# opherlieber/rltime

Measured on AMD Instinct MI355X. Metric: sampled transitions/sec (= learner steps/sec x B x T), IQN-LSTM B=512 T=80 84x84x4, higher is better.
Workload: dtype f32

## Files before the change

include/mirl.h:

```cpp
#ifndef MIRL_H
#define MIRL_H

#include <stdint.h>

#ifdef __cplusplus
extern "C" {
#endif

#define MIRL_OK 0
#define MIRL_NEED_MORE 1
#define MIRL_ERR_ARG (-1)
#define MIRL_ERR_HIP (-2)
#define MIRL_ERR_STATE (-3)
#define MIRL_ERR_NOGPU (-4)

#define MIRL_MODE_UNIFORM 0
#define MIRL_MODE_PER 1

typedef struct mirl_replay mirl_replay;

typedef struct mirl_replay_config {
  int64_t size;
  int32_t num_envs;
  int32_t env_base;
  int32_t frame_bytes;
  int32_t extra_f32;
  int32_t state_f32;
  int32_t has_initials;
  int32_t policy_f32;
  int32_t nstep_train;
  int32_t prefix_steps;
  int32_t nstep_target;
  double  gamma;
  int32_t mode;
  int32_t train_frequency;
  int32_t avoid_episode_crossing;
  int32_t overlap;
  double  alpha, beta, eps, max_weight_factor;
  int32_t beta_anneal_mode;
  double  beta_anneal_to;
  int32_t global_importance_scaling;
  int32_t env_ring_slack;
  int32_t device;
  int32_t acting_priority_init;
  double  acting_vf_eps;
  int32_t stack_planes;
} mirl_replay_config;

typedef struct mirl_ingest {
  int32_t count;
  const int32_t* env_ids_host;
  const uint8_t* frames;
  const float*   extra;
  const float*   state;
  const float*   initials;
  const int32_t* actions;
  const float*   policy;
  const float*   rewards;
  const uint8_t* dones;
  int32_t newest_plane_only;
  int64_t frames_stride;
} mirl_ingest;

typedef struct mirl_batch {
  uint8_t* frames;
  float*   extra;
  float*   state;
  float*   initials;
  float*   returns;
  float*   nsteps;
  float*   masks;
  int64_t* actions;
  float*   policy;
  float*   weights;
  int64_t* loss_indices;
} mirl_batch;

const char* mirl_last_error(void);
int mirl_device_count(void);

int mirl_replay_create(const mirl_replay_config* cfg, mirl_replay** out);
int mirl_replay_destroy(mirl_replay* h);

int mirl_replay_ingest(mirl_replay* h, const mirl_ingest* in, void* stream);
int mirl_replay_ingest_plan(mirl_replay* h, int32_t steps, int32_t count, const int32_t* env_ids_host, void* stream);
int mirl_replay_ingest_planned(mirl_replay* h, int32_t step, const mirl_ingest* in, void* stream);

int mirl_replay_prime_stack(mirl_replay* h, const uint8_t* newest_planes, int64_t stride, void* stream);

int mirl_ingest_fused_set(int32_t on);

int mirl_replay_needed_feed_count(mirl_replay* h, int32_t mbatch, int32_t num_envs, int64_t* out);

int mirl_replay_set_train_quota(mirl_replay* h, int64_t quota);

int mirl_replay_sample(mirl_replay* h, int32_t mbatch, double train_progress,
                       const void* rng_host, uint64_t seed,
                       int32_t* slot, int32_t* env, int64_t* start, int64_t* loss_start,
                       float* weight, double* stats, void* stream);
int mirl_replay_sample_ready(mirl_replay* h, int32_t mbatch, int32_t* ready);
int mirl_replay_sample_skip(mirl_replay* h, int32_t mbatch);
int mirl_replay_tree_root(mirl_replay* h, double* root_dev, void* stream);
int mirl_replay_sample_global(mirl_replay* h, int32_t mbatch_local, int32_t mbatch_global, int32_t rows,
                              int32_t rank, int32_t world, const double* shard_totals,
                              double train_progress, uint64_t seed, int32_t* slot, int32_t* env,
                              int64_t* start, int64_t* loss_start, double* weight_raw,
                              int32_t* stratum, double* stats, void* stream);
int mirl_replay_uniform_total(mirl_replay* h, int64_t* total);

int mirl_replay_state_rows(mirl_replay* h, int32_t* rows, int32_t* overlapped);

int mirl_replay_gather(mirl_replay* h, int32_t mbatch, const int32_t* env,
                       const int64_t* start, const int64_t* loss_start, const float* weight,
                       const mirl_batch* out, void* stream);

int mirl_replay_update_losses(mirl_replay* h, int64_t count, const int64_t* indices,
                              const float* losses, void* stream);

int mirl_replay_save(mirl_replay* h, const char* path_host);
int mirl_replay_load(mirl_replay* h, const char* path_host);

int mirl_replay_profile(mirl_replay* h, int32_t enable, int64_t* launches, double* total_ms);

int mirl_profile_set(int32_t level);
int mirl_profile_collect(int32_t* n_kernels);
int mirl_profile_get(int32_t i, char* name_host, int32_t name_cap, int64_t* calls,
                     double* total_ms, double* algorithmic_bytes);
int mirl_profile_reset(void);
int mirl_profile_get_flop(int32_t i, double* flop);

int mirl_replay_stats(mirl_replay* h, int64_t* total_items, int64_t* active_sequences,
                      int64_t* train_quota, int64_t* tree_capacity, int64_t* n_slots);
int mirl_replay_env_meta(mirl_replay* h, int64_t* first_host, int64_t* count_host);
int mirl_replay_free_slots(mirl_replay* h, int32_t* slots_host, int64_t* n);
int mirl_replay_slot_table(mirl_replay* h, int32_t* slot_env_host, int64_t* slot_base_host);
int mirl_replay_tree_nodes(mirl_replay* h, double* value_host, uint8_t* kind_host, double* min_host);
int mirl_replay_tree_set_leaves(mirl_replay* h, int64_t n, const double* value_host,
                                const uint8_t* kind_host, void* stream);
int mirl_replay_tree_find(mirl_replay* h, int32_t mbatch, const double* uniforms_host,
                          int64_t* idx_host, void* stream);
int mirl_replay_losses_peek(mirl_replay* h, int32_t env_local, int64_t offset, int32_t n, float* out_host);

int mirl_q_target_dqn(int64_t M, int32_t A, const float* q_target, const float* q_select,
                      const float* returns, const float* nsteps, const float* masks,
                      double gamma, double vf_eps, float* targets, void* stream);
int mirl_q_target_iqn(int64_t M, int32_t Nt, int32_t Ns, int32_t A,
                      const float* z_target, const float* z_select,
                      const float* returns, const float* nsteps, const float* masks,
                      double gamma, double vf_eps, float* targets, void* stream);

int mirl_loss_dqn(int64_t M, int32_t A, const float* q, const int64_t* actions,
                  const float* targets, const float* weights, double kappa, int32_t mode,
                  double row_scale, float* row_loss, float* dq, float* td, void* stream);
int mirl_loss_iqn(int64_t M, int32_t N, int32_t Nt, int32_t A, const float* z,
                  const float* taus, const int64_t* actions, const float* targets,
                  const float* weights, double kappa, double row_scale,
                  float* row_loss, float* dz, float* abs_td, void* stream);

int mirl_q_target_c51(int64_t M, int32_t A, int32_t Z, const float* logits_target, const float* logits_select,
                      const float* support, const float* returns, const float* nsteps, const float* masks,
                      double gamma, double vmin, double vmax, double delta_z, int32_t projection,
                      float* targets, void* stream);
int mirl_loss_c51(int64_t M, int32_t A, int32_t Z, const float* logits, const int64_t* actions,
                  const float* targets, const float* weights, int32_t mode, double kappa, double row_scale,
                  float* row_loss, float* dlogits, float* report, void* stream);

int mirl_lstm_cell_fwd(int32_t B, int32_t H, float* gates, const float* c_in, const float* keep_next,
                       float* h_out, float* c_out, float* h_next, float* c_next, void* stream);
int mirl_lstm_seq_supported(int32_t T, int32_t B, int32_t H);
int mirl_lstm_seq_workspace_bytes(int32_t B, int32_t H, int64_t* bytes);
int mirl_lstm_seq_fwd(int32_t T, int32_t B, int32_t H, float* gx, const float* w_hh, const float* h0,
                      const float* c0, const float* keep, float* out, float* c_all, float* hm, float* cm,
                      float* h_last, float* c_last, int32_t save_gates, void* workspace, void* stream);
int mirl_lstm_seq_status(int32_t* status);
int mirl_lstm_seq_fwd_grid(int32_t B, int32_t H, int32_t* workgroups, int64_t* lds_bytes, int32_t* compute_units,
                           int32_t* per_compute_unit);
int mirl_lstm_seq_bwd_supported(int32_t T, int32_t B, int32_t H);
int mirl_lstm_seq_bwd_workspace_bytes(int32_t B, int32_t H, int64_t* bytes);
int mirl_lstm_seq_bwd(int32_t T, int32_t B, int32_t H, float* gates, const float* w_hh, const float* c_all,
                      const float* cm, const float* d_out, const float* keep, void* workspace, void* stream);
int mirl_lstm_cell_bwd(int32_t B, int32_t H, float* gates, const float* c_t, const float* c_in,
                       const float* d_out, const float* dh_rec, float* dc_rec, const float* keep_next,
                       int32_t first, void* stream);

int mirl_frames_to_f32_nhwc(int64_t N, int32_t C, int32_t HW, const uint8_t* src, float scale,
                            float* dst, void* stream);
int mirl_frames_to_f32_nhwc_ex(int64_t N, int32_t C, int32_t HW, const uint8_t* src, float scale,
                               float* dst, int32_t per_wg, int32_t flags, void* stream);

int mirl_conv1_u8_supported(int32_t C, int32_t H, int32_t W, int32_t F, int32_t K, int32_t S);
int mirl_conv1_u8_wpk_floats(int64_t* out);
int mirl_conv1_bf16_set(int32_t mode);
int mirl_conv1_wrw_bf16_set(int32_t mode);
int mirl_conv1_u8_fwd(int64_t N, int32_t H, int32_t W, const uint8_t* x, const float* weight,
                      int64_t ws_o, int64_t ws_c, int64_t ws_h, int64_t ws_w, const float* bias,
                      float scale, float* wpk, float* y, void* stream);
int mirl_conv1_u8_fwd_ex(int64_t N, int32_t H, int32_t W, const uint8_t* x, const float* weight,
                         int64_t ws_o, int64_t ws_c, int64_t ws_h, int64_t ws_w, const float* bias,
                         float scale, float* wpk, float* y, int32_t flags, void* stream);

int mirl_conv1_u8_wrw_scratch_floats(int64_t* out);
int mirl_conv1_u8_wrw(int64_t N, int32_t H, int32_t W, const uint8_t* x, const float* g, float scale,
                      float* scratch, float* dw, int64_t ws_o, int64_t ws_c, int64_t ws_h, int64_t ws_w,
                      void* stream);
int mirl_conv1_u8_wrw_ex(int64_t N, int32_t H, int32_t W, const uint8_t* x, const float* g, float scale,
                         float* scratch, float* dw, int64_t ws_o, int64_t ws_c, int64_t ws_h, int64_t ws_w,
                         int32_t flags, void* stream);
int mirl_conv1_u8_wrw_masked(int64_t N, int32_t H, int32_t W, const uint8_t* x, const float* dy, const float* y, float scale,
                             float* scratch, float* dw, int64_t ws_o, int64_t ws_c, int64_t ws_h, int64_t ws_w,
                             float* db, void* stream);

int mirl_conv2_bwd_data_supported(int32_t C, int32_t F, int32_t K, int32_t S, int32_t IH, int32_t IW,
                                  int32_t OH, int32_t OW);
int mirl_conv2_bwd_data(int64_t N, int32_t OH, int32_t OW, const float* g, const float* weight,
                        int64_t ws_o, int64_t ws_c, int64_t ws_h, int64_t ws_w, float* wpk, float* dx,
                        void* stream);
int mirl_conv2_bwd_data_wpk_floats(int64_t* floats);
int mirl_conv2_bwd_data_ex(int64_t N, int32_t OH, int32_t OW, const float* g, const float* weight, int64_t ws_o,
                           int64_t ws_c, int64_t ws_h, int64_t ws_w, float* wpk, int64_t wpk_floats, float* dx, int32_t pipe,
                           void* stream);
int mirl_conv3_bwd_data_supported(int32_t C, int32_t F, int32_t K, int32_t S, int32_t IH, int32_t IW, int32_t OH, int32_t OW);
int mirl_conv3_bwd_data_wpk_floats(int64_t* floats);
int mirl_conv3_bwd_data(int64_t N, int32_t OH, int32_t OW, const float* g, const float* weight, int64_t ws_o,
                        int64_t ws_c, int64_t ws_h, int64_t ws_w, float* wpk, int64_t wpk_floats, float* dx, void* stream);

int mirl_gemm3_supported(int32_t layout, int64_t M, int64_t N, int64_t K);
int mirl_gemm3_workspace_bytes(int32_t layout, int64_t M, int64_t N, int64_t K, int64_t* bytes);
int mirl_gemm3(int32_t layout, int64_t M, int64_t N, int64_t K, const float* A, int64_t lda,
               const float* B, int64_t ldb, float* C, int64_t ldc, const float* bias, int32_t relu,
               void* workspace, int64_t workspace_bytes, void* stream);
int mirl_gemm3_mid_set(int32_t mode);
int mirl_gemm3_nt_mul(int64_t M, int64_t N, int64_t K, const float* A, int64_t lda, const float* B,
                      int64_t ldb, float* C, int64_t ldc, const float* bias, int32_t relu,
                      const float* mul, int64_t ldmul, int32_t group_shift, float* pre, int64_t ldpre,
                      void* stream);
int mirl_gemm3_head_workspace_bytes(int64_t M, int64_t N, int64_t* bytes);
int mirl_gemm3_nt_head(int64_t M, int64_t N, int64_t K, const float* A, int64_t lda, const float* B, int64_t ldb,
                       float* C, int64_t ldc, const float* bias, int32_t relu, const float* w2, int32_t O,
                       const float* bias2, float* out2, int64_t ldo, void* workspace, int64_t workspace_bytes, void* stream);
int mirl_gemm3_nn_qp_partial_rows(int64_t M, int64_t* rows);
int mirl_gemm3_nn_qp(int64_t M, int64_t N, int64_t K, const float* A, int64_t lda, const float* B, int64_t ldb,
                     const float* emb, int64_t ldemb, const float* x, int64_t ldx, float* d_pre, int64_t ldd,
                     float* dx, int64_t lddx, float* db_partial, void* stream);

int mirl_conv3_fwd_supported(int32_t C, int32_t F, int32_t KH, int32_t KW, int32_t S, int32_t H, int32_t W);
int mirl_conv3_fwd(int64_t N, int32_t H, int32_t W, int32_t C, int32_t F, int32_t KH, int32_t KW, int32_t S,
                   const float* x, const float* w, const float* bias, int32_t relu, float* y, void* stream);

int mirl_conv_wrw_b3_supported(int32_t C, int32_t F, int32_t KH, int32_t KW, int32_t S, int32_t H, int32_t W);
int mirl_conv_wrw_b3_scratch_bytes(int32_t C, int32_t F, int32_t KH, int32_t KW, int64_t* bytes);
int mirl_conv_wrw_b3(int64_t N, int32_t H, int32_t W, int32_t C, int32_t F, int32_t KH, int32_t KW, int32_t S,
                     const float* x, const float* g, void* scratch, int64_t scratch_bytes, float* dw, void* stream);

int mirl_bias_relu_rows(int64_t rows, int32_t C, float* y, const float* bias, void* stream);
int mirl_colsum_blocks(int64_t rows, int32_t C, int32_t* blocks);
int mirl_relu_bwd_bias_rows(int64_t rows, int32_t C, const float* dy, const float* y, float* g,
                            float* db, float* partial, int32_t blocks, void* stream);
int mirl_cos_embed(int64_t rows, int32_t D, const float* tau, const float* freq, float* phi, void* stream);
int mirl_cos_embed_rng(int64_t rows, int32_t D, uint64_t seed, const uint64_t* step, const float* freq,
                       float* phi, float* tau_out, void* stream);
int mirl_iqn_mul_fwd(int64_t M, int32_t N, int32_t C, const float* x, const float* emb, float* out, void* stream);
int mirl_iqn_mul_bwd(int64_t M, int32_t N, int32_t C, const float* g, const float* emb, const float* x,
                     float* d_pre, float* dx, float* db, float* partial, int32_t blocks, void* stream);

int mirl_dueling_tail_bwd(int64_t M, int32_t H1, int32_t Hv, int32_t A, int32_t Q, const float* ga,
                          const float* gv, const float* wo, const float* wq, const float* both,
                          float* g, float* db, float* partial, int32_t blocks, void* stream);
int mirl_dueling_tail_bwd_w(int64_t M, int32_t H1, int32_t Hv, int32_t A, int32_t Q, const float* ga,
                            const float* gv, const float* wo, const float* wq, const float* both, float* g,
                            float* db, float* partial, int32_t blocks, float* dwj, float* partial_w,
                            void* stream);

int mirl_actor_head(int32_t E, int32_t N, int32_t A, const float* adv, const float* val, int32_t Q,
                    const double* eps, const double* expo, double eps_min, const float* u, const int64_t* rnd,
                    int32_t* actions, float* qvalues, float* eps_used, void* stream);
int mirl_actor_head_rng(int32_t E, int32_t N, int32_t A, const float* adv, int32_t adv_pitch, const float* val, int32_t Q,
                        const double* eps, const double* expo, double eps_min, uint64_t rng_seed,
                        const uint64_t* rng_step, int32_t* actions, float* qvalues, float* eps_used, void* stream);
int mirl_actor_head_c51(int32_t E, int32_t A, int32_t Z, const float* adv, int32_t adv_pitch, const float* val,
                        int32_t val_pitch, const float* support, const double* eps, const double* expo, double eps_min,
                        const float* u, const int64_t* rnd, uint64_t rng_seed, const uint64_t* rng_step,
                        int32_t* actions, float* qvalues, float* eps_used, void* stream);
int mirl_stack_shift(int32_t E, int32_t P, int32_t plane_bytes, const uint8_t* in, uint8_t* out,
                     const uint8_t* newest, const uint8_t* dones, void* stream);
#define MIRL_STEP_ADVANCE (~0ull)
int mirl_actor_pre(int32_t E, int32_t H, int32_t A, const float* rewards_raw, const uint8_t* dones,
                   const int32_t* actions, const float* h, const float* c, float* xh_tail, int64_t xh_pitch,
                   float* c_in, float* state_pack, float* initials, float* rewards_out, uint8_t* dones_out,
                   int32_t clip_rewards, float* ep_reward, int32_t* ep_len, float* out_reward, int32_t* out_len,
                   int32_t* action_counts, uint64_t* rng_step, uint64_t step, void* stream);
int mirl_synth_env_step(int32_t E, int64_t frame_bytes, const uint8_t* pool, int32_t pool_n, uint64_t* clock, int32_t slot,
                        uint64_t seed, float p_neg, float p_nonpos, float p_done, uint8_t* obs, float* rewards,
                        uint8_t* dones, void* stream);
int mirl_act_conv_supported(int32_t layer, int32_t Ci, int32_t Co, int32_t k, int32_t stride, int32_t Hi, int32_t Wi);
int mirl_act_conv_fwd(int32_t layer, int64_t frames, int32_t Hi, int32_t Wi, const float* x, const float* w_taps,
                      const float* bias, float* y, int64_t y_frame_pitch, void* stream);
int mirl_act_lstm_supported(int32_t E, int32_t H, int32_t K);
int mirl_act_lstm_workspace_bytes(int32_t E, int32_t H, int32_t K, int64_t* bytes);
int mirl_act_lstm_fwd(int32_t E, int32_t H, int32_t K, const float* xh, int64_t xh_pitch, const float* w, const float* bias,
                      const float* c_in, float* h_out, float* c_out, void* workspace, void* stream);
int mirl_act_embed(int32_t E, int32_t N, int32_t H, int32_t D, const float* h, const float* freq, const float* taus,
                   uint64_t seed, const uint64_t* step, const float* wq, const float* bq, float* x, float* tau_out, void* stream);
int mirl_act_head_supported(int32_t E, int32_t N, int32_t H, int32_t D, int32_t HID, int32_t NO);
int mirl_act_head_parts(int32_t HID, int32_t NO, int32_t* parts, int32_t* pitch);
int mirl_act_head_hidden(int32_t R, int32_t H, int32_t HID, int32_t NO, const float* x, const float* wfc, const float* bfc,
                         const float* wout, float* part, void* stream);
int mirl_act_head_select(int32_t E, int32_t N, int32_t A, int32_t parts, int32_t pitch, const float* part, const float* bout,
                         int32_t has_val, const double* eps, const double* expo, double eps_min, uint64_t rng_seed,
                         const uint64_t* rng_step, int32_t* actions, float* qvalues, void* stream);
int mirl_synth_env_step_pre(int32_t E, int64_t frame_bytes, const uint8_t* pool, int32_t pool_n, uint64_t* clock, int32_t slot,
                            uint64_t seed, float p_neg, float p_nonpos, float p_done, uint8_t* obs, float* rewards,
                            uint8_t* dones, int32_t H, int32_t A, const int32_t* actions, const float* h, const float* c,
                            float* xh_tail, int64_t xh_pitch, float* c_in, float* state_pack, float* initials,
                            float* rewards_out, uint8_t* dones_out, int32_t clip_rewards, float* ep_reward, int32_t* ep_len,
                            float* out_reward, int32_t* out_len, int32_t* action_counts, uint64_t* rng_step, uint64_t step,
                            void* stream);
int mirl_episode_track(int32_t E, int32_t A, const float* rewards, const uint8_t* dones,
                       const int32_t* actions, float* ep_reward, int32_t* ep_len,
                       float* out_reward, int32_t* out_len, int32_t* action_counts, void* stream);

int mirl_copy_bytes(void* dst, const void* src, int64_t bytes, void* stream);
int mirl_copy_bytes_ex(void* dst, const void* src, int64_t bytes, int32_t nt, void* stream);

typedef struct mirl_book mirl_book;
int mirl_book_create(const mirl_replay_config* cfg, mirl_book** out);
int mirl_book_destroy(mirl_book* b);
int mirl_book_ingest(mirl_book* b, int32_t count, const int32_t* env_ids_host);
int mirl_book_stats(mirl_book* b, int64_t* total_items, int64_t* active_sequences,
                    int64_t* train_quota, int64_t* tree_capacity, int64_t* n_slots);
int mirl_book_env_meta(mirl_book* b, int64_t* first_host, int64_t* count_host);
int mirl_book_free_slots(mirl_book* b, int32_t* slots_host, int64_t* n);
int mirl_book_slot_table(mirl_book* b, int32_t* slot_env_host, int64_t* slot_base_host);
int mirl_book_needed_feed_count(mirl_book* b, int32_t mbatch, int32_t num_envs, int64_t* out);
int mirl_book_charge_quota(mirl_book* b, int32_t mbatch);
int mirl_book_uniform_total(mirl_book* b, int64_t* total);
int mirl_book_uniform_map(mirl_book* b, int32_t mbatch, const int64_t* picks_host,
                          int32_t* env_host, int64_t* start_host);
int mirl_emul_build_tree(int64_t capacity, const double* leaf_value, const uint8_t* leaf_kind,
                         double* node_value, uint8_t* node_kind);
int mirl_emul_find(int64_t capacity, const double* node_value, const uint8_t* node_kind,
                   int32_t mbatch, const double* uniforms, int64_t* idx);
int mirl_emul_seq_priority(int32_t nstep_train, double alpha, double max_weight_factor,
                           const float* loss_slots, double* value, uint8_t* kind);

int mirl_adam_clip_workspace_bytes(int32_t count, const int64_t* numel, int64_t* bytes);
int mirl_adam_clip_step(int32_t count, float* const* param, float* const* grad, float* const* exp_avg,
                        float* const* exp_avg_sq, float* const* step, const int64_t* numel, double lr,
                        const float* lr_dev, double beta1, double beta2, double eps, double clip, void* workspace,
                        int64_t workspace_bytes, float* norm_out, void* stream);

#define MIRL_VETO_LOSS 1
#define MIRL_VETO_NORM 2
#define MIRL_VETO_STATUS 4
int mirl_step_guard_open(int32_t* guard, const float* rows, int64_t count, const int32_t* const* status,
                         int32_t n_status, void* stream);
int mirl_adam_clip_step_guarded(int32_t count, float* const* param, float* const* grad, float* const* exp_avg,
                                float* const* exp_avg_sq, float* const* step, const int64_t* numel, double lr,
                                const float* lr_dev, double beta1, double beta2, double eps, double clip, void* workspace,
                                int64_t workspace_bytes, float* norm_out, int32_t* guard, void* stream);
int mirl_replay_update_losses_guarded(mirl_replay* h, int64_t count, const int64_t* indices, const float* losses,
                                      const int32_t* guard, void* stream);
int mirl_lstm_seq_status_device(const int32_t** p);

#ifdef __cplusplus
}
#endif
#endif
```

rltime_amd/_lib.py:

```python
import ctypes as C
import os

import torch

_HERE = os.path.dirname(os.path.abspath(__file__))
LIB_PATH = os.path.join(_HERE, "librltime_hip.so")

MIRL_OK = 0
MIRL_NEED_MORE = 1
MODE_UNIFORM = 0
MODE_PER = 1
INT32_MIN = -2 ** 31


MIRL_OK, MIRL_ERR_ARG, MIRL_ERR_HIP, MIRL_ERR_STATE, MIRL_ERR_NOGPU = 0, -1, -2, -3, -4


class MirlError(RuntimeError):
    code = None


class ReplayConfig(C.Structure):
    _fields_ = [
        ("size", C.c_int64),
        ("num_envs", C.c_int32),
        ("env_base", C.c_int32),
        ("frame_bytes", C.c_int32),
        ("extra_f32", C.c_int32),
        ("state_f32", C.c_int32),
        ("has_initials", C.c_int32),
        ("policy_f32", C.c_int32),
        ("nstep_train", C.c_int32),
        ("prefix_steps", C.c_int32),
        ("nstep_target", C.c_int32),
        ("gamma", C.c_double),
        ("mode", C.c_int32),
        ("train_frequency", C.c_int32),
        ("avoid_episode_crossing", C.c_int32),
        ("overlap", C.c_int32),
        ("alpha", C.c_double),
        ("beta", C.c_double),
        ("eps", C.c_double),
        ("max_weight_factor", C.c_double),
        ("beta_anneal_mode", C.c_int32),
        ("beta_anneal_to", C.c_double),
        ("global_importance_scaling", C.c_int32),
        ("env_ring_slack", C.c_int32),
        ("device", C.c_int32),
        ("acting_priority_init", C.c_int32),
        ("acting_vf_eps", C.c_double),
        ("stack_planes", C.c_int32),
    ]


class Ingest(C.Structure):
    _fields_ = [
        ("count", C.c_int32),
        ("env_ids_host", C.c_void_p),
        ("frames", C.c_void_p),
        ("extra", C.c_void_p),
        ("state", C.c_void_p),
        ("initials", C.c_void_p),
        ("actions", C.c_void_p),
        ("policy", C.c_void_p),
        ("rewards", C.c_void_p),
        ("dones", C.c_void_p),
        ("newest_plane_only", C.c_int32),
        ("frames_stride", C.c_int64),
    ]


class Batch(C.Structure):
    _fields_ = [
        ("frames", C.c_void_p),
        ("extra", C.c_void_p),
        ("state", C.c_void_p),
        ("initials", C.c_void_p),
        ("returns", C.c_void_p),
        ("nsteps", C.c_void_p),
        ("masks", C.c_void_p),
        ("actions", C.c_void_p),
        ("policy", C.c_void_p),
        ("weights", C.c_void_p),
        ("loss_indices", C.c_void_p),
    ]


def _load():
    if not os.path.isfile(LIB_PATH):
        raise MirlError(
            "%s not found: build it with `python -c 'import __graft_entry__ as g; "
            "g.build()'` (rltime_amd/csrc/build.sh). rltime_amd has no CPU "
            "fallback." % LIB_PATH)
    lib = C.CDLL(LIB_PATH)
    lib.mirl_last_error.restype = C.c_char_p
    return lib


lib = _load()

_vp, _i32, _i64, _u64, _f64 = C.c_void_p, C.c_int32, C.c_int64, C.c_uint64, C.c_double
_P = C.POINTER

_SIGNATURES = {
    "mirl_device_count": [],
    "mirl_replay_create": [_P(ReplayConfig), _P(_vp)],
    "mirl_replay_destroy": [_vp],
    "mirl_replay_ingest": [_vp, _P(Ingest), _vp],
    "mirl_replay_ingest_plan": [_vp, _i32, _i32, _vp, _vp],
    "mirl_replay_ingest_planned": [_vp, _i32, _P(Ingest), _vp],
    "mirl_ingest_fused_set": [_i32],
    "mirl_replay_prime_stack": [_vp, _vp, _i64, _vp],
    "mirl_replay_needed_feed_count": [_vp, _i32, _i32, _P(_i64)],
    "mirl_replay_sample": [_vp, _i32, _f64, _vp, _u64, _vp, _vp, _vp, _vp, _vp, _vp, _vp],
    "mirl_replay_sample_ready": [_vp, _i32, _P(_i32)],
    "mirl_replay_sample_skip": [_vp, _i32],
    "mirl_replay_tree_root": [_vp, _vp, _vp],
    "mirl_replay_sample_global": [_vp, _i32, _i32, _i32, _i32, _i32, _vp, _f64, _u64, _vp, _vp, _vp, _vp, _vp, _vp, _vp, _vp],
    "mirl_replay_profile": [_vp, _i32, _P(_i64), _P(_f64)],
    "mirl_profile_set": [_i32],
    "mirl_profile_collect": [_P(_i32)],
    "mirl_profile_get": [_i32, C.c_char_p, _i32, _P(_i64), _P(_f64), _P(_f64)],
    "mirl_profile_get_flop": [_i32, _vp],
    "mirl_profile_reset": [],
    "mirl_replay_save": [_vp, C.c_char_p],
    "mirl_replay_load": [_vp, C.c_char_p],
    "mirl_replay_uniform_total": [_vp, _P(_i64)],
    "mirl_replay_set_train_quota": [_vp, _i64],
    "mirl_replay_state_rows": [_vp, _P(_i32), _P(_i32)],
    "mirl_replay_gather": [_vp, _i32, _vp, _vp, _vp, _vp, _P(Batch), _vp],
    "mirl_replay_update_losses": [_vp, _i64, _vp, _vp, _vp],
    "mirl_replay_stats": [_vp, _P(_i64), _P(_i64), _P(_i64), _P(_i64), _P(_i64)],
    "mirl_replay_env_meta": [_vp, _vp, _vp],
    "mirl_replay_free_slots": [_vp, _vp, _P(_i64)],
    "mirl_replay_slot_table": [_vp, _vp, _vp],
    "mirl_replay_tree_nodes": [_vp, _vp, _vp, _vp],
    "mirl_replay_tree_set_leaves": [_vp, _i64, _vp, _vp, _vp],
    "mirl_replay_tree_find": [_vp, _i32, _vp, _vp, _vp],
    "mirl_replay_losses_peek": [_vp, _i32, _i64, _i32, _vp],
    "mirl_q_target_dqn": [_i64, _i32, _vp, _vp, _vp, _vp, _vp, _f64, _f64, _vp, _vp],
    "mirl_q_target_iqn": [_i64, _i32, _i32, _i32, _vp, _vp, _vp, _vp, _vp, _f64, _f64, _vp, _vp],
    "mirl_loss_dqn": [_i64, _i32, _vp, _vp, _vp, _vp, _f64, _i32, _f64, _vp, _vp, _vp, _vp],
    "mirl_loss_iqn": [_i64, _i32, _i32, _i32, _vp, _vp, _vp, _vp, _vp, _f64, _f64, _vp, _vp, _vp, _vp],
    "mirl_q_target_c51": [_i64, _i32, _i32, _vp, _vp, _vp, _vp, _vp, _vp, _f64, _f64, _f64, _f64, _i32, _vp, _vp],
    "mirl_loss_c51": [_i64, _i32, _i32, _vp, _vp, _vp, _vp, _i32, _f64, _f64, _vp, _vp, _vp, _vp],
    "mirl_actor_head_c51": [_i32, _i32, _i32, _vp, _i32, _vp, _i32, _vp, _vp, _vp, _f64, _vp, _vp, _u64, _vp, _vp, _vp, _vp, _vp],
    "mirl_lstm_cell_fwd": [_i32, _i32, _vp, _vp, _vp, _vp, _vp, _vp, _vp, _vp],
    "mirl_lstm_seq_supported": [_i32, _i32, _i32],
    "mirl_lstm_seq_workspace_bytes": [_i32, _i32, _P(_i64)],
    "mirl_lstm_seq_fwd": [_i32, _i32, _i32, _vp, _vp, _vp, _vp, _vp, _vp, _vp, _vp, _vp, _vp, _vp, _i32, _vp, _vp],
    "mirl_lstm_seq_status": [_P(_i32)],
    "mirl_gemm3_mid_set": [_i32],
    "mirl_lstm_seq_fwd_grid": [_i32, _i32, _P(_i32), _P(_i64), _P(_i32), _P(_i32)],
    "mirl_lstm_seq_bwd_supported": [_i32, _i32, _i32],
    "mirl_lstm_seq_bwd_workspace_bytes": [_i32, _i32, _P(_i64)],
    "mirl_lstm_seq_bwd": [_i32, _i32, _i32, _vp, _vp, _vp, _vp, _vp, _vp, _vp, _vp],
    "mirl_lstm_cell_bwd": [_i32, _i32, _vp, _vp, _vp, _vp, _vp, _vp, _vp, _i32, _vp],
    "mirl_frames_to_f32_nhwc": [_i64, _i32, _i32, _vp, C.c_float, _vp, _vp],
    "mirl_frames_to_f32_nhwc_ex": [_i64, _i32, _i32, _vp, C.c_float, _vp, _i32, _i32, _vp],
    "mirl_conv1_u8_supported": [_i32, _i32, _i32, _i32, _i32, _i32],
    "mirl_conv1_bf16_set": [_i32],
    "mirl_conv1_wrw_bf16_set": [_i32],
    "mirl_conv1_u8_wpk_floats": [_P(_i64)],
    "mirl_conv1_u8_fwd": [_i64, _i32, _i32, _vp, _vp, _i64, _i64, _i64, _i64, _vp, C.c_float, _vp, _vp, _vp],
    "mirl_conv1_u8_fwd_ex": [_i64, _i32, _i32, _vp, _vp, _i64, _i64, _i64, _i64, _vp, C.c_float, _vp, _vp, _i32, _vp],
    "mirl_conv1_u8_wrw_scratch_floats": [_P(_i64)],
    "mirl_conv1_u8_wrw_ex": [_i64, _i32, _i32, _vp, _vp, C.c_float, _vp, _vp, _i64, _i64, _i64, _i64, _i32, _vp],
    "mirl_conv1_u8_wrw_masked": [_i64, _i32, _i32, _vp, _vp, _vp, C.c_float, _vp, _vp, _i64, _i64, _i64, _i64, _vp, _vp],
    "mirl_conv1_u8_wrw": [_i64, _i32, _i32, _vp, _vp, C.c_float, _vp, _vp, _i64, _i64, _i64, _i64, _vp],
    "mirl_conv2_bwd_data_supported": [_i32, _i32, _i32, _i32, _i32, _i32, _i32, _i32],
    "mirl_conv2_bwd_data": [_i64, _i32, _i32, _vp, _vp, _i64, _i64, _i64, _i64, _vp, _vp, _vp],
    "mirl_conv2_bwd_data_wpk_floats": [_P(_i64)],
    "mirl_conv3_bwd_data_supported": [_i32, _i32, _i32, _i32, _i32, _i32, _i32, _i32],
    "mirl_conv3_bwd_data_wpk_floats": [_P(_i64)],
    "mirl_conv3_bwd_data": [_i64, _i32, _i32, _vp, _vp, _i64, _i64, _i64, _i64, _vp, _i64, _vp, _vp],
    "mirl_conv2_bwd_data_ex": [_i64, _i32, _i32, _vp, _vp, _i64, _i64, _i64, _i64, _vp, _i64, _vp, _i32, _vp],
    "mirl_conv3_fwd_supported": [_i32, _i32, _i32, _i32, _i32, _i32, _i32],
    "mirl_conv3_fwd": [_i64, _i32, _i32, _i32, _i32, _i32, _i32, _i32, _vp, _vp, _vp, _i32, _vp, _vp],
    "mirl_conv_wrw_b3_supported": [_i32, _i32, _i32, _i32, _i32, _i32, _i32],
    "mirl_conv_wrw_b3_scratch_bytes": [_i32, _i32, _i32, _i32, _P(_i64)],
    "mirl_conv_wrw_b3": [_i64, _i32, _i32, _i32, _i32, _i32, _i32, _i32, _vp, _vp, _vp, _i64, _vp, _vp],
    "mirl_gemm3_supported": [_i32, _i64, _i64, _i64],
    "mirl_gemm3_workspace_bytes": [_i32, _i64, _i64, _i64, _P(_i64)],
    "mirl_gemm3": [_i32, _i64, _i64, _i64, _vp, _i64, _vp, _i64, _vp, _i64, _vp, _i32, _vp, _i64, _vp],
    "mirl_gemm3_nt_mul": [_i64, _i64, _i64, _vp, _i64, _vp, _i64, _vp, _i64, _vp, _i32, _vp, _i64, _i32, _vp, _i64, _vp],
    "mirl_gemm3_nn_qp_partial_rows": [_i64, _P(_i64)],
    "mirl_gemm3_nn_qp": [_i64, _i64, _i64, _vp, _i64, _vp, _i64, _vp, _i64, _vp, _i64, _vp, _i64, _vp, _i64, _vp, _vp],
    "mirl_gemm3_head_workspace_bytes": [_i64, _i64, _P(_i64)],
    "mirl_gemm3_nt_head": [_i64, _i64, _i64, _vp, _i64, _vp, _i64, _vp, _i64, _vp, _i32, _vp, _i32, _vp, _vp, _i64, _vp, _i64, _vp],
    "mirl_act_conv_supported": [_i32, _i32, _i32, _i32, _i32, _i32, _i32],
    "mirl_act_conv_fwd": [_i32, _i64, _i32, _i32, _vp, _vp, _vp, _vp, _i64, _vp],
    "mirl_act_lstm_supported": [_i32, _i32, _i32],
    "mirl_act_lstm_workspace_bytes": [_i32, _i32, _i32, _P(_i64)],
    "mirl_act_lstm_fwd": [_i32, _i32, _i32, _vp, _i64, _vp, _vp, _vp, _vp, _vp, _vp, _vp],
    "mirl_act_embed": [_i32, _i32, _i32, _i32, _vp, _vp, _vp, _u64, _vp, _vp, _vp, _vp, _vp, _vp],
    "mirl_act_head_supported": [_i32, _i32, _i32, _i32, _i32, _i32],
    "mirl_act_head_parts": [_i32, _i32, _P(_i32), _P(_i32)],
    "mirl_act_head_hidden": [_i32, _i32, _i32, _i32, _vp, _vp, _vp, _vp, _vp, _vp],
    "mirl_act_head_select": [_i32, _i32, _i32, _i32, _i32, _vp, _vp, _i32, _vp, _vp, _f64, _u64, _vp, _vp, _vp, _vp],
    "mirl_bias_relu_rows": [_i64, _i32, _vp, _vp, _vp],
    "mirl_colsum_blocks": [_i64, _i32, _P(_i32)],
    "mirl_relu_bwd_bias_rows": [_i64, _i32, _vp, _vp, _vp, _vp, _vp, _i32, _vp],
    "mirl_cos_embed": [_i64, _i32, _vp, _vp, _vp, _vp],
    "mirl_cos_embed_rng": [_i64, _i32, _u64, _vp, _vp, _vp, _vp, _vp],
    "mirl_adam_clip_workspace_bytes": [_i32, _vp, _vp],
    "mirl_adam_clip_step": [_i32, _vp, _vp, _vp, _vp, _vp, _vp, _f64, _vp, _f64, _f64, _f64, _f64, _vp, _i64, _vp, _vp],
    "mirl_adam_clip_step_guarded": [_i32, _vp, _vp, _vp, _vp, _vp, _vp, _f64, _vp, _f64, _f64, _f64, _f64, _vp, _i64, _vp, _vp, _vp],
    "mirl_step_guard_open": [_vp, _vp, _i64, _vp, _i32, _vp],
    "mirl_replay_update_losses_guarded": [_vp, _i64, _vp, _vp, _vp, _vp],
    "mirl_lstm_seq_status_device": [_P(_vp)],
    "mirl_iqn_mul_fwd": [_i64, _i32, _i32, _vp, _vp, _vp, _vp],
    "mirl_iqn_mul_bwd": [_i64, _i32, _i32, _vp, _vp, _vp, _vp, _vp, _vp, _vp, _i32, _vp],
    "mirl_dueling_tail_bwd": [_i64, _i32, _i32, _i32, _i32, _vp, _vp, _vp, _vp, _vp, _vp, _vp, _vp, _i32, _vp],
    "mirl_dueling_tail_bwd_w": [_i64, _i32, _i32, _i32, _i32, _vp, _vp, _vp, _vp, _vp, _vp, _vp, _vp, _i32, _vp, _vp, _vp],
    "mirl_actor_head": [_i32, _i32, _i32, _vp, _vp, _i32, _vp, _vp, _f64, _vp, _vp, _vp, _vp, _vp, _vp],
    "mirl_actor_head_rng": [_i32, _i32, _i32, _vp, _i32, _vp, _i32, _vp, _vp, _f64, _u64, _vp, _vp, _vp, _vp, _vp],
    "mirl_stack_shift": [_i32, _i32, _i32, _vp, _vp, _vp, _vp, _vp],
    "mirl_synth_env_step": [_i32, _i64, _vp, _i32, _vp, _i32, _u64, C.c_float, C.c_float, C.c_float, _vp, _vp, _vp, _vp],
    "mirl_synth_env_step_pre": [_i32, _i64, _vp, _i32, _vp, _i32, _u64, C.c_float, C.c_float, C.c_float, _vp, _vp, _vp,
                                _i32, _i32, _vp, _vp, _vp, _vp, _i64, _vp, _vp, _vp, _vp, _vp, _i32, _vp, _vp, _vp, _vp, _vp, _vp, _u64, _vp],
    "mirl_actor_pre": [_i32, _i32, _i32, _vp, _vp, _vp, _vp, _vp, _vp, _i64, _vp, _vp, _vp, _vp, _vp, _i32, _vp, _vp, _vp, _vp,
                       _vp, _vp, _u64, _vp],
    "mirl_episode_track": [_i32, _i32, _vp, _vp, _vp, _vp, _vp, _vp, _vp, _vp, _vp],
    "mirl_copy_bytes": [_vp, _vp, _i64, _vp],
    "mirl_copy_bytes_ex": [_vp, _vp, _i64, _i32, _vp],
    "mirl_book_create": [_P(ReplayConfig), _P(_vp)],
    "mirl_book_destroy": [_vp],
    "mirl_book_ingest": [_vp, _i32, _vp],
    "mirl_book_stats": [_vp, _P(_i64), _P(_i64), _P(_i64), _P(_i64), _P(_i64)],
    "mirl_book_env_meta": [_vp, _vp, _vp],
    "mirl_book_free_slots": [_vp, _vp, _P(_i64)],
    "mirl_book_slot_table": [_vp, _vp, _vp],
    "mirl_book_needed_feed_count": [_vp, _i32, _i32, _P(_i64)],
    "mirl_book_charge_quota": [_vp, _i32],
    "mirl_book_uniform_total": [_vp, _P(_i64)],
    "mirl_book_uniform_map": [_vp, _i32, _vp, _vp, _vp],
    "mirl_emul_build_tree": [_i64, _vp, _vp, _vp, _vp],
    "mirl_emul_find": [_i64, _vp, _vp, _i32, _vp, _vp],
    "mirl_emul_seq_priority": [_i32, _f64, _f64, _vp, _P(_f64), _P(C.c_uint8)],
}

for _name, _args in _SIGNATURES.items():
    _fn = getattr(lib, _name)
    _fn.argtypes = _args
    _fn.restype = C.c_int


def last_error():
    return (lib.mirl_last_error() or b"").decode()


def check(rc, what=""):
    if rc < 0:
        err = MirlError("%s failed (%d): %s" % (what or "mirl call", rc, last_error()))
        err.code = int(rc)
        raise err
    return rc


def ptr(t):
    return C.c_void_p(t.data_ptr() if t is not None else None)


def stream():
    return C.c_void_p(torch.cuda.current_stream().cuda_stream)


def device_count():
    return lib.mirl_device_count()


def require_gpu():
    if device_count() <= 0:
        raise MirlError(
            "librltime_hip: no HIP device visible. The rltime_amd hot path runs "
            "only on an AMD GPU (MI355X / gfx950); there is no CPU fallback.")


def profile_table():
    n = C.c_int32()
    check(lib.mirl_profile_collect(C.byref(n)), "mirl_profile_collect")
    out = []
    for i in range(n.value):
        name = C.create_string_buffer(96)
        calls, ms, by = C.c_int64(), C.c_double(), C.c_double()
        check(lib.mirl_profile_get(i, name, 96, C.byref(calls), C.byref(ms), C.byref(by)), "mirl_profile_get")
        fl = C.c_double()
        check(lib.mirl_profile_get_flop(i, C.byref(fl)), "mirl_profile_get_flop")
        out.append({"name": name.value.decode(), "calls": calls.value, "total_ms": ms.value,
                    "algorithmic_bytes": by.value, "flop": fl.value})
    return out


def np_ptr(a):
    return a.ctypes.data_as(C.c_void_p)
```

rltime_amd/csrc/conv_mid.hip:

```cpp
#include "common.hpp"
#include "split3.hpp"
#include <stdlib.h>

namespace mirl {

typedef float cm_f4 __attribute__((ext_vector_type(4)));

constexpr int C2_C = 32, C2_F = 64, C2_K = 4, C2_S = 2;
constexpr int C2_STEPS = 64;
constexpr int C2_WPK = 4 * 2 * C2_STEPS * 64;
constexpr int C2_PP = 68;
constexpr int C2_LD = 6;

__global__ void __launch_bounds__(256)
k_conv2_pack_w(const float* __restrict__ w, int64_t so, int64_t sc, int64_t sh, int64_t sw, float* __restrict__ wpk) {
  const int t = blockIdx.x * 256 + threadIdx.x;
  if (t >= C2_WPK) return;
  const int lane = t & 63, s = (t >> 6) & 63, m = (t >> 12) & 1, cls = t >> 13;
  const int i = lane & 15, kq = lane >> 4;
  const int f = kq * 16 + (s & 15), kh = (cls >> 1) + 2 * (s >> 5), kw = (cls & 1) + 2 * ((s >> 4) & 1);
  const int c = (i >> 2) * 8 + m * 4 + (i & 3);
  wpk[t] = w[f * so + c * sc + kh * sh + kw * sw];
}

template <int FPI>
__global__ void __launch_bounds__(256, 2)
k_conv2_bwd_data(int N, int OH, int OW, unsigned v_magic, const float* __restrict__ g,
                 const float* __restrict__ wpk, float* __restrict__ dx) {
  extern __shared__ __align__(16) float c2_lds[];
  const int tid = threadIdx.x, lane = tid & 63, cls = __builtin_amdgcn_readfirstlane(tid >> 6);
  const int j = lane & 15, kq = lane >> 4;
  const int ph = cls >> 1, pw = cls & 1;
  float wr0[C2_STEPS], wr1[C2_STEPS];
#pragma unroll
  for (int s = 0; s < C2_STEPS; ++s) {
    wr0[s] = wpk[((cls * 2 + 0) * C2_STEPS + s) * 64 + lane];
    wr1[s] = wpk[((cls * 2 + 1) * C2_STEPS + s) * 64 + lane];
  }
  const int PW = OW + 2, rows = FPI * (OH + 1) + 1;
  const int U = OH + 1, V = OW + 1, UV = U * V, IH = 2 * OH + 2, IW = 2 * OW + 2;
  const int pos16 = OH * OW * 16;
  for (int o = tid; o < rows * PW * (C2_PP / 4); o += 256) reinterpret_cast<cm_f4*>(c2_lds)[o] = cm_f4{0.f, 0.f, 0.f, 0.f};
  const int units = (N + FPI - 1) / FPI;
  for (int u0 = blockIdx.x; u0 < units; u0 += gridDim.x) {
    const int n0 = u0 * FPI;
    const int frames = N - n0 < FPI ? N - n0 : FPI;
    __syncthreads();
    {
      const int vecs = frames * pos16;
      const cm_f4* s4 = reinterpret_cast<const cm_f4*>(g + (int64_t)n0 * OH * OW * C2_F);
      for (int o0 = tid; o0 < vecs; o0 += 256 * C2_LD) {
        cm_f4 v[C2_LD];
#pragma unroll
        for (int k = 0; k < C2_LD; ++k) { const int o = o0 + k * 256; v[k] = s4[o < vecs ? o : vecs - 1]; }
#pragma unroll
        for (int k = 0; k < C2_LD; ++k) {
          const int o = o0 + k * 256;
          if (o < vecs) {
            const int f = o >= pos16 ? 1 : 0, r = o - f * pos16, pos = r >> 4, sub = r & 15;
            const int oh2 = pos / OW, ow2 = pos - oh2 * OW;
            *reinterpret_cast<cm_f4*>(c2_lds + ((f * (OH + 1) + 1 + oh2) * PW + 1 + ow2) * C2_PP + sub * 4) = v[k];
          }
        }
      }
    }
    __syncthreads();
    const int pend = frames * UV;
    for (int p0 = 0; p0 < pend; p0 += 16) {
      const int p = p0 + j, pc = p < pend ? p : pend - 1;
      const int f = (FPI > 1 && pc >= UV) ? 1 : 0, r = pc - f * UV;
      const int u = V == 1 ? r : (int)__umulhi((unsigned)r, v_magic), v = r - u * V;
      const float* base = c2_lds + ((f * (OH + 1) + 1 + u) * PW + 1 + v) * C2_PP + kq * 16;
      cm_f4 gq[16];
#pragma unroll
      for (int ab = 0; ab < 4; ++ab) {
        const float* pb = base - ((ab >> 1) * PW + (ab & 1)) * C2_PP;
#pragma unroll
        for (int e = 0; e < 4; ++e) gq[ab * 4 + e] = *reinterpret_cast<const cm_f4*>(pb + e * 4);
      }
      cm_f4 a0 = {0.f, 0.f, 0.f, 0.f}, a1 = {0.f, 0.f, 0.f, 0.f};
#pragma unroll
      for (int s = 0; s < C2_STEPS; ++s) {
        const float val = gq[s >> 2][s & 3];
        a0 = __builtin_amdgcn_mfma_f32_16x16x4f32(wr0[s], val, a0, 0, 0, 0);
        a1 = __builtin_amdgcn_mfma_f32_16x16x4f32(wr1[s], val, a1, 0, 0, 0);
      }
      if (p < pend) {
        cm_f4* dst = reinterpret_cast<cm_f4*>(dx + ((((int64_t)(n0 + f) * IH + 2 * u + ph) * IW) + 2 * v + pw) * C2_C + kq * 8);
        dst[0] = a0; dst[1] = a1;
      }
    }
  }
}

static size_t c2_lds_bytes(int fpi, int OH, int OW) { return (size_t)(fpi * (OH + 1) + 1) * (OW + 2) * C2_PP * 4; }

constexpr int C2B_SLOTS = 4 * 2 * 8;
constexpr int C2B_PF = 6;
constexpr int C2B_WPK_BYTES = C2B_SLOTS * 3 * 64 * 16;

__host__ __device__ inline int c2b_chunk_stride(int npos) { return ((npos + 15) / 16) * 256 + 16; }
__host__ __device__ inline int c2b_half_plane(int npos) { return (4 * c2b_chunk_stride(npos) + 255) / 256 * 256; }

__global__ void __launch_bounds__(256)
k_conv2_pack_w3b(const float* __restrict__ w, int64_t so, int64_t sc, int64_t sh, int64_t sw, uint4* __restrict__ wpk3) {
  const int t = blockIdx.x * 256 + threadIdx.x;
  if (t >= C2B_SLOTS * 64) return;
  const int lane = t & 63, slot = t >> 6, st = slot & 7, m = (slot >> 3) & 1, cls = slot >> 4;
  const int c = 16 * m + (lane & 15), tap = st >> 1;
  const int kh = (cls >> 1) + 2 * (tap >> 1), kw = (cls & 1) + 2 * (tap & 1);
  const int f0 = 32 * (st & 1) + 8 * (lane >> 4);
  float x[2][4];
#pragma unroll
  for (int e = 0; e < 8; ++e) x[e >> 2][e & 3] = w[(f0 + e) * so + c * sc + kh * sh + kw * sw];
  uint2 h0, m0, l0, h1, m1, l1;
  g3_split4(x[0], h0, m0, l0);
  g3_split4(x[1], h1, m1, l1);
  wpk3[(slot * 3 + 0) * 64 + lane] = make_uint4(h0.x, h0.y, h1.x, h1.y);
  wpk3[(slot * 3 + 1) * 64 + lane] = make_uint4(m0.x, m0.y, m1.x, m1.y);
  wpk3[(slot * 3 + 2) * 64 + lane] = make_uint4(l0.x, l0.y, l1.x, l1.y);
}

template <int FPI>
__global__ void __launch_bounds__(512) __attribute__((amdgpu_waves_per_eu(2, 2)))
k_conv2_bwd_data_b3(int N, int OH, int OW, unsigned v_magic, const float* __restrict__ g,
                    const uint4* __restrict__ wpk3, float* __restrict__ dx) {
  extern __shared__ __align__(16) char c2b_lds[];
  const int tid = threadIdx.x, lane = tid & 63, wave = __builtin_amdgcn_readfirstlane(tid >> 6);
  const int cls = wave >> 1, m = wave & 1;
  const int j = lane & 15, kq = lane >> 4;
  const int ph = cls >> 1, pw = cls & 1;
  g3_bf16x8 wr[8][3];
#pragma unroll
  for (int s = 0; s < 8; ++s)
#pragma unroll
    for (int p = 0; p < 3; ++p)
      wr[s][p] = __builtin_bit_cast(g3_bf16x8, wpk3[((((cls * 2 + m) * 8 + s) * 3) + p) * 64 + lane]);
  const int PW = OW + 2, rows = FPI * (OH + 1) + 1;
  const int U = OH + 1, V = OW + 1, UV = U * V, IH = 2 * OH + 2, IW = 2 * OW + 2;
  const int pos16 = OH * OW * 16;
  const int S = c2b_chunk_stride(rows * PW), HP = c2b_half_plane(rows * PW), plane = 2 * HP;
  for (int o = tid; o < 3 * plane / 16; o += 512) reinterpret_cast<uint4*>(c2b_lds)[o] = make_uint4(0u, 0u, 0u, 0u);
  const int units = (N + FPI - 1) / FPI;
  constexpr int PF = C2B_PF;
  const bool pf = FPI * pos16 <= 512 * PF;
  cm_f4 nv[PF];
  auto request = [&](int unit) {
    const int nn0 = unit * FPI;
    const int vecs = (N - nn0 < FPI ? N - nn0 : FPI) * pos16;
    const cm_f4* s4 = reinterpret_cast<const cm_f4*>(g + (int64_t)nn0 * OH * OW * C2_F);
#pragma unroll
    for (int k = 0; k < PF; ++k) { const int o = tid + k * 512; nv[k] = s4[o < vecs ? o : vecs - 1]; }
  };
  auto put = [&](const cm_f4& val, int o) {
    const int f = o >= pos16 ? 1 : 0, r = o - f * pos16, pos = r >> 4, sub = r & 15;
    const int oh2 = pos / OW, ow2 = pos - oh2 * OW;
    const float x[4] = {val.x, val.y, val.z, val.w};
    uint2 hh, mm, ll;
    g3_split4(x, hh, mm, ll);
    const int chunk = sub >> 1, kqw = chunk & 3;
    char* d = c2b_lds + (kqw & 1) * HP + (2 * (chunk >> 2) + (kqw >> 1)) * S + ((f * (OH + 1) + 1 + oh2) * PW + 1 + ow2) * 16 + (sub & 1) * 8;
    *reinterpret_cast<uint2*>(d) = hh;
    *reinterpret_cast<uint2*>(d + plane) = mm;
    *reinterpret_cast<uint2*>(d + 2 * plane) = ll;
  };
  if (pf && (int)blockIdx.x < units) request(blockIdx.x);
  for (int u0 = blockIdx.x; u0 < units; u0 += gridDim.x) {
    const int n0 = u0 * FPI;
    const int frames = N - n0 < FPI ? N - n0 : FPI;
    __syncthreads();
    {
      const int vecs = frames * pos16;
      if (pf) {
#pragma unroll
        for (int k = 0; k < PF; ++k) { const int o = tid + k * 512; if (o < vecs) put(nv[k], o); }
      } else {
        const cm_f4* s4 = reinterpret_cast<const cm_f4*>(g + (int64_t)n0 * OH * OW * C2_F);
        constexpr int LD = 4;
        for (int o0 = tid; o0 < vecs; o0 += 512 * LD) {
          cm_f4 v[LD];
#pragma unroll
          for (int k = 0; k < LD; ++k) { const int o = o0 + k * 512; v[k] = s4[o < vecs ? o : vecs - 1]; }
#pragma unroll
          for (int k = 0; k < LD; ++k) { const int o = o0 + k * 512; if (o < vecs) put(v[k], o); }
        }
      }
    }
    if (pf && u0 + (int)gridDim.x < units) request(u0 + gridDim.x);
    g3_barrier();
    const int pend = frames * UV;
    int f, u, v;
    auto locate = [&](int p0) -> const char* {
      const int p = p0 + j, pc = p < pend ? p : pend - 1;
      f = (FPI > 1 && pc >= UV) ? 1 : 0;
      const int r = pc - f * UV;
      u = V == 1 ? r : (int)__umulhi((unsigned)r, v_magic);
      v = r - u * V;
      return c2b_lds + (kq & 1) * HP + (kq >> 1) * S + ((f * (OH + 1) + 1 + u) * PW + 1 + v) * 16;
    };
    auto load_half = [&](g3_bf16x8 (&b)[4][3], const char* base, int hs) {
#pragma unroll
      for (int q = 0; q < 4; ++q) {
        const int s = hs * 4 + q;
        const char* pb = base - (((s >> 2) & 1) * PW + ((s >> 1) & 1)) * 16 + (s & 1) * 2 * S;
        b[q][0] = *reinterpret_cast<const g3_bf16x8*>(pb);
        b[q][1] = *reinterpret_cast<const g3_bf16x8*>(pb + plane);
        b[q][2] = *reinterpret_cast<const g3_bf16x8*>(pb + 2 * plane);
      }
    };
    auto mfma_half = [&](g3_f32x4 acc, const g3_bf16x8 (&b)[4][3], int hs) -> g3_f32x4 {
#pragma unroll
      for (int q = 0; q < 4; ++q) {
        const int s = hs * 4 + q;
        acc = __builtin_amdgcn_mfma_f32_16x16x32_bf16(wr[s][2], b[q][0], acc, 0, 0, 0);
        acc = __builtin_amdgcn_mfma_f32_16x16x32_bf16(wr[s][0], b[q][2], acc, 0, 0, 0);
        acc = __builtin_amdgcn_mfma_f32_16x16x32_bf16(wr[s][1], b[q][1], acc, 0, 0, 0);
        acc = __builtin_amdgcn_mfma_f32_16x16x32_bf16(wr[s][1], b[q][0], acc, 0, 0, 0);
        acc = __builtin_amdgcn_mfma_f32_16x16x32_bf16(wr[s][0], b[q][1], acc, 0, 0, 0);
        acc = __builtin_amdgcn_mfma_f32_16x16x32_bf16(wr[s][0], b[q][0], acc, 0, 0, 0);
      }
      return acc;
    };
    g3_bf16x8 b0[4][3], b1[4][3];
    const char* base = locate(0);
    load_half(b0, base, 0);
    for (int p0 = 0; p0 < pend; p0 += 16) {
      load_half(b1, base, 1);
      float* dst = dx + ((((int64_t)(n0 + f) * IH + 2 * u + ph) * IW) + 2 * v + pw) * C2_C + 16 * m + 4 * kq;
      const bool live = p0 + j < pend;
      __builtin_amdgcn_sched_barrier(0);
      g3_f32x4 acc = {0.f, 0.f, 0.f, 0.f};
      acc = mfma_half(acc, b0, 0);
      __builtin_amdgcn_sched_barrier(0);
      if (p0 + 16 < pend) {
        base = locate(p0 + 16);
        load_half(b0, base, 0);
      }
      __builtin_amdgcn_sched_barrier(0);
      acc = mfma_half(acc, b1, 1);
      __builtin_amdgcn_sched_barrier(0);
      if (live) *reinterpret_cast<g3_f32x4*>(dst) = acc;
    }
  }
}

static size_t c2b_lds_bytes(int fpi, int OH, int OW) { return (size_t)3 * 2 * c2b_half_plane((fpi * (OH + 1) + 1) * (OW + 2)); }

constexpr int C3B_C = 64, C3B_F = 64, C3B_K = 3;
constexpr int C3B_HS = 9;
constexpr int C3B_SLOTS = 4 * 2 * C3B_HS;
constexpr int C3B_WPK_BYTES = C3B_SLOTS * 3 * 64 * 16;
constexpr int C3B_MAXT = 11;

__global__ void __launch_bounds__(256)
k_conv3_pack_w3b(const float* __restrict__ w, int64_t so, int64_t sc, int64_t sh, int64_t sw, uint4* __restrict__ wpk3) {
  const int t = blockIdx.x * 256 + threadIdx.x;
  if (t >= C3B_SLOTS * 64) return;
  const int lane = t & 63, slot = t >> 6, q = slot % C3B_HS, kh2 = (slot / C3B_HS) & 1, ct = slot / (2 * C3B_HS);
  const int st = kh2 * C3B_HS + q, tap = st >> 1, kh = tap / C3B_K, kw = tap - kh * C3B_K;
  const int c = 16 * ct + (lane & 15), f0 = 32 * (st & 1) + 8 * (lane >> 4);
  float x[2][4];
#pragma unroll
  for (int e = 0; e < 8; ++e) x[e >> 2][e & 3] = w[(f0 + e) * so + c * sc + kh * sh + kw * sw];
  uint2 h0, m0, l0, h1, m1, l1;
  g3_split4(x[0], h0, m0, l0);
  g3_split4(x[1], h1, m1, l1);
  wpk3[(slot * 3 + 0) * 64 + lane] = make_uint4(h0.x, h0.y, h1.x, h1.y);
  wpk3[(slot * 3 + 1) * 64 + lane] = make_uint4(m0.x, m0.y, m1.x, m1.y);
  wpk3[(slot * 3 + 2) * 64 + lane] = make_uint4(l0.x, l0.y, l1.x, l1.y);
}

template <int FPI>
__global__ void __launch_bounds__(512) __attribute__((amdgpu_waves_per_eu(2, 2)))
k_conv3_bwd_data_b3(int N, int OH, int OW, unsigned iw_magic, const float* __restrict__ g, const uint4* __restrict__ wpk3,
                    float* __restrict__ dx) {
  extern __shared__ __align__(16) char c3b_lds[];
  const int tid = threadIdx.x, lane = tid & 63, wave = __builtin_amdgcn_readfirstlane(tid >> 6);
  const int ct = wave >> 1, kh2 = wave & 1;
  const int j = lane & 15, kq = lane >> 4;
  g3_bf16x8 wr[C3B_HS][3];
#pragma unroll
  for (int q = 0; q < C3B_HS; ++q)
#pragma unroll
    for (int p = 0; p < 3; ++p)
      wr[q][p] = __builtin_bit_cast(g3_bf16x8, wpk3[((((ct * 2 + kh2) * C3B_HS + q) * 3) + p) * 64 + lane]);
  const int IH = OH + 2, IW = OW + 2, IHW = IH * IW, PW = OW + 4, rows = FPI * (OH + 2) + 2;
  const int pos16 = OH * OW * 16;
  const int S = c2b_chunk_stride(rows * PW), HP = c2b_half_plane(rows * PW), plane = 2 * HP;
  int tsh[C3B_HS], fsh[C3B_HS];
#pragma unroll
  for (int q = 0; q < C3B_HS; ++q) {
    const int st = kh2 * C3B_HS + q, tap = st >> 1, kh = tap / C3B_K, kw = tap - kh * C3B_K;
    tsh[q] = (kh * PW + kw) * 16;
    fsh[q] = (st & 1) * 2 * S;
  }
  for (int o = tid; o < 3 * plane / 16; o += 512) reinterpret_cast<uint4*>(c3b_lds)[o] = make_uint4(0u, 0u, 0u, 0u);
  const int units = (N + FPI - 1) / FPI;
  bool first = true;
  for (int u0 = blockIdx.x; u0 < units; u0 += gridDim.x) {
    const int n0 = u0 * FPI;
    const int frames = N - n0 < FPI ? N - n0 : FPI;
    __syncthreads();
    if (!first) {
      for (int o = tid; o < 4 * C3B_MAXT * 64; o += 512) reinterpret_cast<uint4*>(c3b_lds)[o] = make_uint4(0u, 0u, 0u, 0u);
      __syncthreads();
    }
    first = false;
    {
      const int vecs = frames * pos16;
      const cm_f4* s4 = reinterpret_cast<const cm_f4*>(g + (int64_t)n0 * OH * OW * C3B_F);
      constexpr int LD = 4;
      for (int o0 = tid; o0 < vecs; o0 += 512 * LD) {
        cm_f4 v[LD];
#pragma unroll
        for (int k = 0; k < LD; ++k) { const int o = o0 + k * 512; v[k] = s4[o < vecs ? o : vecs - 1]; }
#pragma unroll
        for (int k = 0; k < LD; ++k) {
          const int o = o0 + k * 512;
          if (o < vecs) {
            const int f = o / pos16, r = o - f * pos16, pos = r >> 4, sub = r & 15;
            const int oh2 = pos / OW, ow2 = pos - oh2 * OW;
            const float x[4] = {v[k].x, v[k].y, v[k].z, v[k].w};
            uint2 hh, mm, ll;
            g3_split4(x, hh, mm, ll);
            const int chunk = sub >> 1, kqw = chunk & 3;
            char* d = c3b_lds + (kqw & 1) * HP + (2 * (chunk >> 2) + (kqw >> 1)) * S + ((f * (OH + 2) + 2 + oh2) * PW + 2 + ow2) * 16 + (sub & 1) * 8;
            *reinterpret_cast<uint2*>(d) = hh;
            *reinterpret_cast<uint2*>(d + plane) = mm;
            *reinterpret_cast<uint2*>(d + 2 * plane) = ll;
          }
        }
      }
    }
    __syncthreads();
    const int pend = frames * IHW;
    g3_f32x4 acc[C3B_MAXT];
#pragma unroll
    for (int t = 0; t < C3B_MAXT; ++t) {
      acc[t] = g3_f32x4{0.f, 0.f, 0.f, 0.f};
      if (t * 16 < pend) {
        const int p = t * 16 + j, pc = p < pend ? p : pend - 1;
        const int f = pc / IHW, r = pc - f * IHW;
        const int y = (int)__umulhi((unsigned)r, iw_magic), x = r - y * IW;
        const char* base = c3b_lds + (kq & 1) * HP + (kq >> 1) * S + ((f * (OH + 2) + 2 + y) * PW + 2 + x) * 16;
        g3_bf16x8 b[C3B_HS][3];
#pragma unroll
        for (int q = 0; q < C3B_HS; ++q) {
          const char* pb = base - tsh[q] + fsh[q];
          b[q][0] = *reinterpret_cast<const g3_bf16x8*>(pb);
          b[q][1] = *reinterpret_cast<const g3_bf16x8*>(pb + plane);
          b[q][2] = *reinterpret_cast<const g3_bf16x8*>(pb + 2 * plane);
        }
        g3_f32x4 a = {0.f, 0.f, 0.f, 0.f};
#pragma unroll
        for (int q = 0; q < C3B_HS; ++q) {
          a = __builtin_amdgcn_mfma_f32_16x16x32_bf16(wr[q][2], b[q][0], a, 0, 0, 0);
          a = __builtin_amdgcn_mfma_f32_16x16x32_bf16(wr[q][0], b[q][2], a, 0, 0, 0);
          a = __builtin_amdgcn_mfma_f32_16x16x32_bf16(wr[q][1], b[q][1], a, 0, 0, 0);
          a = __builtin_amdgcn_mfma_f32_16x16x32_bf16(wr[q][1], b[q][0], a, 0, 0, 0);
          a = __builtin_amdgcn_mfma_f32_16x16x32_bf16(wr[q][0], b[q][1], a, 0, 0, 0);
          a = __builtin_amdgcn_mfma_f32_16x16x32_bf16(wr[q][0], b[q][0], a, 0, 0, 0);
        }
        acc[t] = a;
      }
    }
    __syncthreads();
    g3_f32x4* xb = reinterpret_cast<g3_f32x4*>(c3b_lds) + (ct * C3B_MAXT) * 64 + lane;
    if (kh2 == 1) {
#pragma unroll
      for (int t = 0; t < C3B_MAXT; ++t) if (t * 16 < pend) xb[t * 64] = acc[t];
    }
    __syncthreads();
    if (kh2 == 0) {
#pragma unroll
      for (int t = 0; t < C3B_MAXT; ++t) {
        const int p = t * 16 + j;
        if (p < pend) {
          const int f = p / IHW, r = p - f * IHW;
          *reinterpret_cast<g3_f32x4*>(dx + ((int64_t)(n0 + f) * IHW + r) * C3B_C + 16 * ct + 4 * kq) = acc[t] + xb[t * 64];
        }
      }
    }
  }
}

static size_t c3b_lds_bytes(int fpi, int OH, int OW) {
  const size_t planes = (size_t)3 * 2 * c2b_half_plane((fpi * (OH + 2) + 2) * (OW + 4)), xchg = (size_t)4 * C3B_MAXT * 1024;
  return planes > xchg ? planes : xchg;
}

struct BwdDataLaunch {
  const char *pack_name, *name;
  double pack_bytes, bytes, flop;
  unsigned pack_grid;
  int fpi;
  size_t lds, lds_limit;
  int grid_cap, block, magic_div;
};
template <typename WPK>
static int bwd_data_launch(const BwdDataLaunch& c, void (*pack)(const float*, int64_t, int64_t, int64_t, int64_t, WPK*),
                           void (*k2)(int, int, int, unsigned, const float*, const WPK*, float*),
                           void (*k1)(int, int, int, unsigned, const float*, const WPK*, float*), int64_t N, int32_t OH, int32_t OW,
                           const float* g, const float* weight, int64_t ws_o, int64_t ws_c, int64_t ws_h, int64_t ws_w, float* wpk,
                           float* dx, hipStream_t st) {
  {
    ProfScope ps(c.pack_name, c.pack_bytes, st);
    hipLaunchKernelGGL(pack, dim3(c.pack_grid), dim3(256), 0, st, weight, ws_o, ws_c, ws_h, ws_w, reinterpret_cast<WPK*>(wpk));
    MIRL_LAUNCH_CHECK();
  }
  const auto k = c.fpi == 2 ? k2 : k1;
  if (c.lds_limit) { if (int rc = raise_lds_limit(k, c.lds_limit)) return rc; }
  ProfScope ps(c.name, c.bytes, st, c.flop);
  hipLaunchKernelGGL(k, dim3(capped_grid((N + c.fpi - 1) / c.fpi, c.grid_cap)), dim3(c.block), c.lds, st, (int)N, OH, OW,
                     magic_u32(c.magic_div), g, reinterpret_cast<const WPK*>(wpk), dx);
  MIRL_LAUNCH_CHECK();
  return MIRL_OK;
}

}

extern "C" int mirl_conv2_bwd_data_supported(int32_t C, int32_t F, int32_t K, int32_t S, int32_t IH, int32_t IW, int32_t OH, int32_t OW) {
  using namespace mirl;
  if (C != C2_C || F != C2_F || K != C2_K || S != C2_S || OH < 1 || OW < 1) return 0;
  if (IH != 2 * OH + 2 || IW != 2 * OW + 2) return 0;
  return c2_lds_bytes(1, OH, OW) <= 64 * 1024 ? 1 : 0;
}

extern "C" int mirl_conv2_bwd_data(int64_t N, int32_t OH, int32_t OW, const float* g, const float* weight, int64_t ws_o,
                                   int64_t ws_c, int64_t ws_h, int64_t ws_w, float* wpk, float* dx, void* stream) {
  using namespace mirl;
  if (N <= 0 || N >= (1LL << 30) || !g || !weight || !wpk || !dx) return fail(MIRL_ERR_ARG, "bad conv2_bwd_data arguments");
  if (!mirl_conv2_bwd_data_supported(C2_C, C2_F, C2_K, C2_S, 2 * OH + 2, 2 * OW + 2, OH, OW))
    return fail(MIRL_ERR_ARG, "conv2_bwd_data: unsupported shape");
  if (!aligned16(g, dx, wpk)) return fail(MIRL_ERR_ARG, "conv2_bwd_data: pointers must be 16-byte aligned");
  BwdDataLaunch c;
  c.pack_name = "k_conv2_pack_w"; c.pack_bytes = 2.0 * C2_WPK * 4; c.pack_grid = (C2_WPK + 255) / 256;
  c.fpi = (N >= 1024 && c2_lds_bytes(2, OH, OW) <= 64 * 1024) ? 2 : 1;
  c.lds = c2_lds_bytes(c.fpi, OH, OW); c.lds_limit = 0;
  c.grid_cap = 512; c.block = 256; c.magic_div = OW + 1;
  c.name = "k_conv2_bwd_data"; c.bytes = (double)N * ((double)OH * OW * C2_F * 4 + (double)(2 * OH + 2) * (2 * OW + 2) * C2_C * 4);
  c.flop = (double)N * OH * OW * 2.0 * C2_K * C2_K * C2_C * C2_F;
  return bwd_data_launch<float>(c, k_conv2_pack_w, k_conv2_bwd_data<2>, k_conv2_bwd_data<1>, N, OH, OW, g, weight, ws_o, ws_c, ws_h, ws_w, wpk,
                                dx, (hipStream_t)stream);
}

extern "C" int mirl_conv2_bwd_data_wpk_floats(int64_t* floats) {
  if (!floats) return mirl::fail(MIRL_ERR_ARG, "conv2_bwd_data_wpk_floats: null out");
  *floats = mirl::C2B_WPK_BYTES / 4 > mirl::C2_WPK ? mirl::C2B_WPK_BYTES / 4 : mirl::C2_WPK;
  return MIRL_OK;
}

extern "C" int mirl_conv2_bwd_data_ex(int64_t N, int32_t OH, int32_t OW, const float* g, const float* weight, int64_t ws_o,
                                      int64_t ws_c, int64_t ws_h, int64_t ws_w, float* wpk, int64_t wpk_floats, float* dx, int32_t pipe, void* stream) {
  using namespace mirl;
  if (wpk_floats < (pipe == 1 ? C2B_WPK_BYTES / 4 : C2_WPK)) return fail(MIRL_ERR_ARG, "conv2_bwd_data_ex: wpk smaller than mirl_conv2_bwd_data_wpk_floats()");
  if (pipe == 0) return mirl_conv2_bwd_data(N, OH, OW, g, weight, ws_o, ws_c, ws_h, ws_w, wpk, dx, stream);
  if (pipe != 1) return fail(MIRL_ERR_ARG, "conv2_bwd_data_ex: pipe is 0 (f32) or 1 (split bf16)");
  if (N <= 0 || N >= (1LL << 30) || !g || !weight || !wpk || !dx) return fail(MIRL_ERR_ARG, "bad conv2_bwd_data arguments");
  if (!mirl_conv2_bwd_data_supported(C2_C, C2_F, C2_K, C2_S, 2 * OH + 2, 2 * OW + 2, OH, OW) || c2b_lds_bytes(1, OH, OW) > 160 * 1024)
    return fail(MIRL_ERR_ARG, "conv2_bwd_data: unsupported shape");
  if (!aligned16(g, dx, wpk)) return fail(MIRL_ERR_ARG, "conv2_bwd_data: pointers must be 16-byte aligned");
  BwdDataLaunch c;
  c.pack_name = "k_conv2_pack_w3b"; c.pack_bytes = 4.0 * C2_WPK + C2B_WPK_BYTES; c.pack_grid = (C2B_SLOTS * 64 + 255) / 256;
  c.fpi = (N >= 512 && c2b_lds_bytes(2, OH, OW) <= 160 * 1024) ? 2 : 1;
  c.lds = c2b_lds_bytes(c.fpi, OH, OW); c.lds_limit = 160 * 1024;
  c.grid_cap = 256; c.block = 512; c.magic_div = OW + 1;
  c.name = "k_conv2_bwd_data_b3"; c.bytes = (double)N * ((double)OH * OW * C2_F * 4 + (double)(2 * OH + 2) * (2 * OW + 2) * C2_C * 4);
  c.flop = (double)N * OH * OW * 2.0 * C2_K * C2_K * C2_C * C2_F;
  return bwd_data_launch<uint4>(c, k_conv2_pack_w3b, k_conv2_bwd_data_b3<2>, k_conv2_bwd_data_b3<1>, N, OH, OW, g, weight, ws_o, ws_c, ws_h, ws_w,
                                wpk, dx, (hipStream_t)stream);
}


extern "C" int mirl_conv3_bwd_data_supported(int32_t C, int32_t F, int32_t K, int32_t S, int32_t IH, int32_t IW, int32_t OH, int32_t OW) {
  using namespace mirl;
  if (C != C3B_C || F != C3B_F || K != C3B_K || S != 1 || OH < 1 || OW < 1) return 0;
  if (IH != OH + 2 || IW != OW + 2) return 0;
  if (IH * IW > 16 * C3B_MAXT) return 0;
  return c3b_lds_bytes(1, OH, OW) <= 150 * 1024 ? 1 : 0;
}

extern "C" int mirl_conv3_bwd_data_wpk_floats(int64_t* floats) {
  if (!floats) return mirl::fail(MIRL_ERR_ARG, "conv3_bwd_data_wpk_floats: null out");
  *floats = mirl::C3B_WPK_BYTES / 4;
  return MIRL_OK;
}

extern "C" int mirl_conv3_bwd_data(int64_t N, int32_t OH, int32_t OW, const float* g, const float* weight, int64_t ws_o,
                                   int64_t ws_c, int64_t ws_h, int64_t ws_w, float* wpk, int64_t wpk_floats, float* dx, void* stream) {
  using namespace mirl;
  if (N <= 0 || N >= (1LL << 30) || !g || !weight || !wpk || !dx) return fail(MIRL_ERR_ARG, "bad conv3_bwd_data arguments");
  if (wpk_floats < C3B_WPK_BYTES / 4) return fail(MIRL_ERR_ARG, "conv3_bwd_data: wpk smaller than mirl_conv3_bwd_data_wpk_floats()");
  if (!mirl_conv3_bwd_data_supported(C3B_C, C3B_F, C3B_K, 1, OH + 2, OW + 2, OH, OW)) return fail(MIRL_ERR_ARG, "conv3_bwd_data: unsupported shape");
  if (!aligned16(g, dx, wpk)) return fail(MIRL_ERR_ARG, "conv3_bwd_data: pointers must be 16-byte aligned");
  const int IHW = (OH + 2) * (OW + 2);
  BwdDataLaunch c;
  c.pack_name = "k_conv3_pack_w3b"; c.pack_bytes = 4.0 * C3B_F * C3B_C * 9 + C3B_WPK_BYTES; c.pack_grid = (C3B_SLOTS * 64 + 255) / 256;
  c.fpi = (N >= 512 && 2 * IHW <= 16 * C3B_MAXT && c3b_lds_bytes(2, OH, OW) <= 150 * 1024) ? 2 : 1;
  c.lds = c3b_lds_bytes(c.fpi, OH, OW); c.lds_limit = 150 * 1024;
  c.grid_cap = 256; c.block = 512; c.magic_div = OW + 2;
  c.name = "k_conv3_bwd_data_b3"; c.bytes = (double)N * 4.0 * C3B_F * ((double)OH * OW + (double)IHW);
  c.flop = (double)N * OH * OW * 2.0 * C3B_K * C3B_K * C3B_C * C3B_F;
  return bwd_data_launch<uint4>(c, k_conv3_pack_w3b, k_conv3_bwd_data_b3<2>, k_conv3_bwd_data_b3<1>, N, OH, OW, g, weight, ws_o, ws_c, ws_h, ws_w,
                                wpk, dx, (hipStream_t)stream);
}
```

rltime_amd/csrc/gemm3.hip:

```cpp
#include "common.hpp"
#include "split3.hpp"
#include <stdlib.h>

namespace mirl {

struct G3Args {
  const float* A; const float* B; float* C; const float* bias;
  int64_t M, N, K;
  int64_t lda, ldb, ldc;
  int relu;
  int mt, nt;
  int splits;
  int steps_per_split;
  const float* mul; int64_t ldmul; int mul_shift;
  float* pre; int64_t ldpre;
  int vec_ok;
  const float* w2; float* part;
  float* gsum; int64_t ldgsum;
};


template <bool KC>
struct G3Loader {
  const float* p[2];
  int64_t step;
  int64_t ld;
  int lds_off;
  __device__ __forceinline__ void init(const float* base, int64_t ld_, int64_t row0, int64_t rows, int64_t k0, int t) {
    ld = ld_;
    if (KC) {
      const int r = t >> 2, kq = t & 3;
#pragma unroll
      for (int h = 0; h < 2; ++h) {
        int64_t row = row0 + r + 128 * h; if (row > rows - 1) row = rows - 1;
        p[h] = base + row * ld + k0 + kq * 4;
      }
      step = 16;
      lds_off = r * G3_PITCH + kq * 8;
    } else {
      const int kq = t >> 7, r = t & 127;
#pragma unroll
      for (int h = 0; h < 2; ++h) {
        int64_t row = row0 + r + 128 * h; if (row > rows - 1) row = rows - 1;
        p[h] = base + (k0 + kq * 4) * ld + row;
      }
      step = 16 * ld;
      lds_off = r * G3_PITCH + kq * 8;
    }
  }
  __device__ __forceinline__ void load(float (&v)[2][4]) {
#pragma unroll
    for (int h = 0; h < 2; ++h) {
      if (KC) {
        const float4 q = *reinterpret_cast<const float4*>(p[h]);
        v[h][0] = q.x; v[h][1] = q.y; v[h][2] = q.z; v[h][3] = q.w;
      } else {
#pragma unroll
        for (int e = 0; e < 4; ++e) v[h][e] = p[h][e * ld];
      }
      p[h] += step;
    }
  }
  __device__ __forceinline__ void store(char* planes, const float (&v)[2][4]) const {
#pragma unroll
    for (int h = 0; h < 2; ++h) {
      uint2 a, b, c;
      g3_split4(v[h], a, b, c);
      char* d = planes + lds_off + h * 128 * G3_PITCH;
      *reinterpret_cast<uint2*>(d) = a;
      *reinterpret_cast<uint2*>(d + G3_PLANE) = b;
      *reinterpret_cast<uint2*>(d + 2 * G3_PLANE) = c;
    }
  }
};

template <int TI>
__device__ __forceinline__ void g3_compute(const char* stage, g3_f32x16 (&acc)[TI][2], int a_off, int b_off) {
  const char* pa = stage + a_off;
  const char* pb = stage + 3 * G3_PLANE + b_off;
  constexpr int PA[6] = {2, 0, 1, 1, 0, 0};
  constexpr int PB[6] = {0, 2, 1, 0, 1, 0};
  g3_bf16x8 b[3][2];
#pragma unroll
  for (int p = 0; p < 3; ++p)
#pragma unroll
    for (int j = 0; j < 2; ++j) b[p][j] = *reinterpret_cast<const g3_bf16x8*>(pb + p * G3_PLANE + j * 32 * G3_PITCH);
  constexpr int IW = TI >= 2 ? 2 : 1;
#pragma unroll
  for (int ih = 0; ih < TI / IW; ++ih) {
    g3_bf16x8 a[3][IW];
#pragma unroll
    for (int p = 0; p < 3; ++p)
#pragma unroll
      for (int i = 0; i < IW; ++i) a[p][i] = *reinterpret_cast<const g3_bf16x8*>(pa + p * G3_PLANE + (ih * IW + i) * 32 * G3_PITCH);
#pragma unroll
    for (int c = 0; c < 6; ++c)
#pragma unroll
      for (int i = 0; i < IW; ++i)
#pragma unroll
        for (int j = 0; j < 2; ++j) acc[ih * IW + i][j] = g3_mfma(a[PA[c]][i], b[PB[c]][j], acc[ih * IW + i][j]);
  }
}


template <bool AKC, bool BKC, int EP, bool VEC, bool NARROW = false>
__global__ void __launch_bounds__(512)
k_gemm3(G3Args g) {
  constexpr int TI = NARROW ? 1 : 4;
  extern __shared__ __attribute__((aligned(16))) char g3_lds[];
  const int t = threadIdx.x, lane = t & 63, wave = t >> 6;
  const int b = blockIdx.x, xcd = b & 7, l = b >> 3, L = gridDim.x >> 3;
  const int64_t nk_all = g.K / 16;
  const int E = g.splits > 1 ? l + 1 : ((g.mt + 7) / 8) * g.nt;
  int split = 0;
  int64_t ks0 = 0, nk = nk_all;

  const int wu = __builtin_amdgcn_readfirstlane(wave);
  const int wm = NARROW ? 0 : (wu & 1), wn = NARROW ? 0 : (wu >> 1);
  const int row_w = NARROW ? wu * 32 : wm * 128;
  const int a_off = (row_w + (lane & 31)) * G3_PITCH + (lane >> 5) * 16;
  const int b_off = (wn * 64 + (lane & 31)) * G3_PITCH + (lane >> 5) * 16;
  const bool stage_first = (wu >> 2) & 1;

  int e = l, it = 0, jt = 0;
  if (g.splits > 1) {
    const int tiles = g.mt * g.nt, tile = l % tiles;
    split = xcd + 8 * (l / tiles);
    it = tile / g.nt; jt = tile % g.nt;
    ks0 = (int64_t)split * g.steps_per_split;
    nk = nk_all - ks0; if (nk > g.steps_per_split) nk = g.steps_per_split;
    if (nk < 0) nk = 0;
  } else {
    for (; e < E; e += L) { jt = e % g.nt; it = (e / g.nt) * 8 + xcd; if (it < g.mt) break; }
    if (e >= E) return;
  }

  G3Loader<AKC> la; G3Loader<BKC> lb;
  float va[2][4], vb[2][4];
  la.init(g.A, g.lda, (int64_t)it * 256, g.M, ks0 * 16, t);
  lb.init(g.B, g.ldb, (int64_t)jt * 256, g.N, ks0 * 16, t);
  if (nk > 0) { la.load(va); lb.load(vb); }

  g3_f32x16 acc[TI][2];
  while (true) {
    const int64_t m0 = (int64_t)it * 256, n0 = (int64_t)jt * 256;
#pragma unroll
    for (int i = 0; i < TI; ++i)
#pragma unroll
      for (int j = 0; j < 2; ++j)
#pragma unroll
        for (int r = 0; r < 16; ++r) acc[i][j][r] = 0.0f;

    if (nk > 0) {
      la.store(g3_lds, va); lb.store(g3_lds + 3 * G3_PLANE, vb);
      if (nk > 1) { la.load(va); lb.load(vb); }
    }
    g3_barrier();
    for (int64_t k = 0; k < nk; ++k) {
      const char* cur = g3_lds + (k & 1) * G3_STAGE;
      char* nxt = g3_lds + ((k + 1) & 1) * G3_STAGE;
      if (stage_first) {
        if (k + 1 < nk) { la.store(nxt, va); lb.store(nxt + 3 * G3_PLANE, vb); }
        if (k + 2 < nk) { la.load(va); lb.load(vb); }
      }
      __builtin_amdgcn_s_setprio(1);
      g3_compute<TI>(cur, acc, a_off, b_off);
      __builtin_amdgcn_s_setprio(0);
      if (!stage_first) {
        if (k + 1 < nk) { la.store(nxt, va); lb.store(nxt + 3 * G3_PLANE, vb); }
        if (k + 2 < nk) { la.load(va); lb.load(vb); }
      }
      g3_barrier();
    }

    bool more = false;
    if (g.splits <= 1) {
      for (e += L; e < E; e += L) { jt = e % g.nt; it = (e / g.nt) * 8 + xcd; if (it < g.mt) break; }
      more = e < E;
      if (more) {
        la.init(g.A, g.lda, (int64_t)it * 256, g.M, 0, t);
        lb.init(g.B, g.ldb, (int64_t)jt * 256, g.N, 0, t);
        la.load(va); lb.load(vb);
      }
    }

    float* C = g.C + (g.splits > 1 ? (int64_t)split * g.M * g.N : 0);
    if (VEC) {
      float* tl = reinterpret_cast<float*>(g3_lds) + wu * (64 * G3_EPITCH);
      constexpr int HALVES = NARROW ? 1 : 2, II = NARROW ? 1 : 2, QN = NARROW ? 8 : 16;
      float* w2l = reinterpret_cast<float*>(g3_lds) + 8 * (64 * G3_EPITCH);
      float bj[2] = {0.f, 0.f};
      g3_f32x4 sb = {0.f, 0.f, 0.f, 0.f};
      if (EP == 2) {
        const int64_t wc = n0 + (t & 63) * 4;
        float4 w = make_float4(0.f, 0.f, 0.f, 0.f);
        if (wc < g.N) w = *reinterpret_cast<const float4*>(g.w2 + (int64_t)(t >> 6) * g.N + wc);
        *reinterpret_cast<float4*>(w2l + (t >> 6) * 256 + (t & 63) * 4) = w;
#pragma unroll
        for (int j = 0; j < 2; ++j) {
          const int64_t cj = n0 + wn * 64 + j * 32 + (lane & 31);
          bj[j] = (g.bias && cj < g.N) ? g.bias[cj] : 0.f;
        }
#pragma unroll
        for (int i = 0; i < TI; ++i)
#pragma unroll
          for (int j = 0; j < 2; ++j)
#pragma unroll
            for (int r = 0; r < 16; ++r) {
              float v = acc[i][j][r] + bj[j];
              acc[i][j][r] = (g.relu && !(v > 0.f)) ? 0.f : v;
            }
        g3_barrier();
      }
#pragma unroll
      for (int h = 0; h < HALVES; ++h) {
#pragma unroll
        for (int ii = 0; ii < II; ++ii)
#pragma unroll
          for (int j = 0; j < 2; ++j)
#pragma unroll
            for (int r = 0; r < 16; ++r)
              tl[(ii * 32 + (r & 3) + 8 * (r >> 2) + 4 * (lane >> 5)) * G3_EPITCH + j * 32 + (lane & 31)] = acc[II * h + ii][j][r];
        asm volatile("s_waitcnt lgkmcnt(0)" ::: "memory");
        const int c4 = lane & 15;
        const int64_t col = n0 + wn * 64 + c4 * 4;
        float4 bv = make_float4(0.f, 0.f, 0.f, 0.f);
        if (EP != 2 && g.bias && col < g.N) {
          bv = *reinterpret_cast<const float4*>(g.bias + col);
        }
        if (EP == 2) {
          const int rg = lane & 15, cq = lane >> 4;
          const int64_t cb = (n0 >> 6) + wn;
#pragma unroll 1
          for (int ip = 0; ip < 2; ++ip) {
            float ps[2][8];
#pragma unroll
            for (int i = 0; i < 2; ++i)
#pragma unroll
              for (int o = 0; o < 8; ++o) ps[i][o] = 0.f;
#pragma unroll 1
            for (int c = 0; c < 4; ++c) {
              asm volatile("" ::: "memory");
              float4 dv[2];
#pragma unroll
              for (int i = 0; i < 2; ++i) dv[i] = *reinterpret_cast<const float4*>(tl + (rg + 16 * (2 * ip + i)) * G3_EPITCH + cq * 16 + c * 4);
#pragma unroll
              for (int o = 0; o < 8; ++o) {
                const float4 w = *reinterpret_cast<const float4*>(w2l + o * 256 + wn * 64 + cq * 16 + c * 4);
#pragma unroll
                for (int i = 0; i < 2; ++i)
                  ps[i][o] = fmaf(dv[i].w, w.w, fmaf(dv[i].z, w.z, fmaf(dv[i].y, w.y, fmaf(dv[i].x, w.x, ps[i][o]))));
              }
            }
#pragma unroll
            for (int i = 0; i < 2; ++i)
#pragma unroll
              for (int o = 0; o < 8; ++o) {
                float v = ps[i][o];
                v += __shfl_xor(v, 16);
                v += __shfl_xor(v, 32);
                ps[i][o] = v;
              }
            if (cq == 0) {
#pragma unroll
              for (int i = 0; i < 2; ++i) {
                const int64_t row = m0 + row_w + h * 64 + rg + 16 * (2 * ip + i);
                if (row < g.M) {
                  float* d = g.part + (cb * g.M + row) * 8;
                  *reinterpret_cast<float4*>(d) = make_float4(ps[i][0], ps[i][1], ps[i][2], ps[i][3]);
                  *reinterpret_cast<float4*>(d + 4) = make_float4(ps[i][4], ps[i][5], ps[i][6], ps[i][7]);
                }
              }
            }
          }
        }
        float4 mg0 = make_float4(0.f, 0.f, 0.f, 0.f), mg1 = mg0;
        const bool hoisted = (EP == 1 && g.mul_shift >= 5) || EP == 3;
        if ((EP == 1 || EP == 3) && hoisted) {
          const int64_t rb = m0 + row_w + h * 64 + (lane >> 4);
          const int64_t r0 = rb < g.M ? rb : g.M - 1, r1 = rb + 32 < g.M ? rb + 32 : g.M - 1;
          const int64_t cc = col < g.N ? col : 0;
          mg0 = *reinterpret_cast<const float4*>(g.mul + (r0 >> g.mul_shift) * g.ldmul + cc);
          mg1 = *reinterpret_cast<const float4*>(g.mul + (r1 >> g.mul_shift) * g.ldmul + cc);
        }
        if (EP == 3) {
          const float4 mgs[2] = {mg0, mg1};
#pragma unroll
          for (int gq = 0; gq < 2; ++gq) {
            g3_f32x4 ev[8];
#pragma unroll
            for (int u = 0; u < 8; ++u) {
              const int64_t row = m0 + row_w + h * 64 + (gq * 8 + u) * 4 + (lane >> 4);
              const int64_t rr = row < g.M ? row : g.M - 1, cc = col < g.N ? col : 0;
              ev[u] = __builtin_nontemporal_load(reinterpret_cast<const g3_f32x4*>(g.pre + rr * g.ldpre + cc));
            }
            g3_f32x4 sg = {0.f, 0.f, 0.f, 0.f};
            const g3_f32x4 xm = {mgs[gq].x, mgs[gq].y, mgs[gq].z, mgs[gq].w};
#pragma unroll
            for (int u = 0; u < 8; ++u) {
              const int rl = (gq * 8 + u) * 4 + (lane >> 4);
              const int64_t row = m0 + row_w + h * 64 + rl;
              const float4 t4 = *reinterpret_cast<const float4*>(tl + rl * G3_EPITCH + c4 * 4);
              const g3_f32x4 v = {t4.x, t4.y, t4.z, t4.w};
              if (row < g.M && col < g.N) {
                g3_f32x4 d = v * xm;
                d.x = ev[u].x > 0.f ? d.x : 0.f; d.y = ev[u].y > 0.f ? d.y : 0.f;
                d.z = ev[u].z > 0.f ? d.z : 0.f; d.w = ev[u].w > 0.f ? d.w : 0.f;
                __builtin_nontemporal_store(d, reinterpret_cast<g3_f32x4*>(C + row * g.ldc + col));
                sg += v * ev[u];
                sb += d;
              }
            }
#pragma unroll
            for (int e = 0; e < 4; ++e) {
              float v = sg[e];
              v += __shfl_xor(v, 16);
              v += __shfl_xor(v, 32);
              sg[e] = v;
            }
            const int64_t row0 = m0 + row_w + h * 64 + gq * 32;
            if ((lane >> 4) == 0 && row0 < g.M && col < g.N)
              *reinterpret_cast<g3_f32x4*>(g.gsum + (row0 >> 5) * g.ldgsum + col) = sg;
          }
        }
#pragma unroll
        for (int q = 0; q < QN; ++q) {
          const int rl = q * 4 + (lane >> 4);
          const int64_t row = m0 + row_w + h * 64 + rl;
          if (EP == 3) break;
          if (EP == 2 && !g.C) break;
          float4 v = *reinterpret_cast<const float4*>(tl + rl * G3_EPITCH + c4 * 4);
          if (row < g.M && col < g.N) {
            if (EP != 2) {
              v.x += bv.x; v.y += bv.y; v.z += bv.z; v.w += bv.w;
              if (g.relu) { v.x = v.x > 0.f ? v.x : 0.f; v.y = v.y > 0.f ? v.y : 0.f; v.z = v.z > 0.f ? v.z : 0.f; v.w = v.w > 0.f ? v.w : 0.f; }
            }
            if (EP == 1) {
              if (g.pre) __builtin_nontemporal_store(g3_f32x4{v.x, v.y, v.z, v.w}, reinterpret_cast<g3_f32x4*>(g.pre + row * g.ldpre + col));
              float4 m;
              if (hoisted) m = q < 8 ? mg0 : mg1;
              else m = *reinterpret_cast<const float4*>(g.mul + (row >> g.mul_shift) * g.ldmul + col);
              v.x *= m.x; v.y *= m.y; v.z *= m.z; v.w *= m.w;
            }
            __builtin_nontemporal_store(g3_f32x4{v.x, v.y, v.z, v.w}, reinterpret_cast<g3_f32x4*>(C + row * g.ldc + col));
          }
        }
        asm volatile("s_waitcnt lgkmcnt(0)" ::: "memory");
      }
      if (EP == 3) {
#pragma unroll
        for (int e = 0; e < 4; ++e) {
          float v = sb[e];
          v += __shfl_xor(v, 16);
          v += __shfl_xor(v, 32);
          sb[e] = v;
        }
        const int64_t col = n0 + wn * 64 + (lane & 15) * 4;
        if ((lane >> 4) == 0 && col < g.N)
          *reinterpret_cast<g3_f32x4*>(g.part + ((m0 >> 8) * 2 + wm) * g.N + col) = sb;
      }
      if (more) g3_barrier();
    } else {
#pragma unroll
      for (int j = 0; j < 2; ++j) {
        const int64_t col = n0 + wn * 64 + j * 32 + (lane & 31);
        const bool col_ok = col < g.N;
        const float bv = (g.bias && col_ok) ? g.bias[col] : 0.0f;
#pragma unroll
        for (int i = 0; i < TI; ++i) {
          const int64_t rb = m0 + row_w + i * 32 + 4 * (lane >> 5);
#pragma unroll
          for (int r = 0; r < 16; ++r) {
            const int64_t row = rb + (r & 3) + 8 * (r >> 2);
            if (!(col_ok && row < g.M)) continue;
            float v = acc[i][j][r] + bv;
            if (g.relu) v = v > 0.0f ? v : 0.0f;
            if (EP == 1) {
              if (g.pre) __builtin_nontemporal_store(v, g.pre + row * g.ldpre + col);
              v *= g.mul[(row >> g.mul_shift) * g.ldmul + col];
            }
            __builtin_nontemporal_store(v, C + row * g.ldc + col);
          }
        }
      }
    }
    if (!more) break;
  }
}


constexpr int G3M_BROWS = 128;
constexpr int G3M_BPLANE = G3M_BROWS * G3_PITCH;
constexpr int G3M_STAGE = 3 * G3_PLANE + 3 * G3M_BPLANE;
constexpr int G3M_LDS = 2 * G3M_STAGE;
constexpr int G3M_EPITCH = 36;

__global__ void __launch_bounds__(512)
k_gemm3_mid(G3Args g) {
  extern __shared__ __attribute__((aligned(16))) char g3_lds[];
  const int t = threadIdx.x, lane = t & 63;
  const int wu = __builtin_amdgcn_readfirstlane(t >> 6);
  const int wm = wu & 1, wn = wu >> 1;
  const int b = blockIdx.x, xcd = b & 7, l = b >> 3;
  const int jt = l % g.nt, it = (l / g.nt) * 8 + xcd;
  if (it >= g.mt) return;
  const int64_t m0 = (int64_t)it * 256, n0 = (int64_t)jt * G3M_BROWS;
  const int64_t nk = g.K / 16;

  G3Loader<true> la;
  la.init(g.A, g.lda, m0, g.M, 0, t);
  const int rb = t >> 2, kq = t & 3;
  int64_t brow = n0 + rb; if (brow > g.N - 1) brow = g.N - 1;
  const float* pb = g.B + brow * g.ldb + kq * 4;
  const int b_lds = rb * G3_PITCH + kq * 8;
  float va[2][4], vb[4];
  auto load_b = [&]() { const float4 q = *reinterpret_cast<const float4*>(pb); vb[0] = q.x; vb[1] = q.y; vb[2] = q.z; vb[3] = q.w; pb += 16; };
  auto store_b = [&](char* planes) {
    uint2 h, m, lo;
    g3_split4(vb, h, m, lo);
    *reinterpret_cast<uint2*>(planes + b_lds) = h;
    *reinterpret_cast<uint2*>(planes + G3M_BPLANE + b_lds) = m;
    *reinterpret_cast<uint2*>(planes + 2 * G3M_BPLANE + b_lds) = lo;
  };
  const int a_off = (wm * 128 + (lane & 31)) * G3_PITCH + (lane >> 5) * 16;
  const int b_off = (wn * 32 + (lane & 31)) * G3_PITCH + (lane >> 5) * 16;
  const bool stage_first = (wu >> 2) & 1;

  g3_f32x16 acc[4];
#pragma unroll
  for (int i = 0; i < 4; ++i)
#pragma unroll
    for (int r = 0; r < 16; ++r) acc[i][r] = 0.0f;
  constexpr int PA[6] = {2, 0, 1, 1, 0, 0};
  constexpr int PB[6] = {0, 2, 1, 0, 1, 0};

  if (nk > 0) { la.load(va); load_b(); la.store(g3_lds, va); store_b(g3_lds + 3 * G3_PLANE); }
  if (nk > 1) { la.load(va); load_b(); }
  g3_barrier();
  for (int64_t k = 0; k < nk; ++k) {
    const char* cur = g3_lds + (k & 1) * G3M_STAGE;
    char* nxt = g3_lds + ((k + 1) & 1) * G3M_STAGE;
    if (stage_first) {
      if (k + 1 < nk) { la.store(nxt, va); store_b(nxt + 3 * G3_PLANE); }
      if (k + 2 < nk) { la.load(va); load_b(); }
    }
    {
      const char* pa = cur + a_off;
      const char* pbf = cur + 3 * G3_PLANE + b_off;
      g3_bf16x8 bf[3];
#pragma unroll
      for (int p = 0; p < 3; ++p) bf[p] = *reinterpret_cast<const g3_bf16x8*>(pbf + p * G3M_BPLANE);
      __builtin_amdgcn_s_setprio(1);
#pragma unroll
      for (int ih = 0; ih < 2; ++ih) {
        g3_bf16x8 a[3][2];
#pragma unroll
        for (int p = 0; p < 3; ++p)
#pragma unroll
          for (int i = 0; i < 2; ++i) a[p][i] = *reinterpret_cast<const g3_bf16x8*>(pa + p * G3_PLANE + (ih * 2 + i) * 32 * G3_PITCH);
#pragma unroll
        for (int c = 0; c < 6; ++c)
#pragma unroll
          for (int i = 0; i < 2; ++i) acc[ih * 2 + i] = g3_mfma(a[PA[c]][i], bf[PB[c]], acc[ih * 2 + i]);
      }
      __builtin_amdgcn_s_setprio(0);
    }
    if (!stage_first) {
      if (k + 1 < nk) { la.store(nxt, va); store_b(nxt + 3 * G3_PLANE); }
      if (k + 2 < nk) { la.load(va); load_b(); }
    }
    g3_barrier();
  }

  float* tl = reinterpret_cast<float*>(g3_lds) + wu * (32 * G3M_EPITCH);
  const int c4 = lane & 7;
  const int64_t col = n0 + wn * 32 + c4 * 4;
  float4 bv = make_float4(0.f, 0.f, 0.f, 0.f);
  if (g.bias && col < g.N) bv = *reinterpret_cast<const float4*>(g.bias + col);
#pragma unroll
  for (int i = 0; i < 4; ++i) {
#pragma unroll
    for (int r = 0; r < 16; ++r)
      tl[((r & 3) + 8 * (r >> 2) + 4 * (lane >> 5)) * G3M_EPITCH + (lane & 31)] = acc[i][r];
    asm volatile("s_waitcnt lgkmcnt(0)" ::: "memory");
#pragma unroll
    for (int q = 0; q < 4; ++q) {
      const int rl = q * 8 + (lane >> 3);
      const int64_t row = m0 + wm * 128 + i * 32 + rl;
      float4 v = *reinterpret_cast<const float4*>(tl + rl * G3M_EPITCH + c4 * 4);
      if (row < g.M && col < g.N) {
        v.x += bv.x; v.y += bv.y; v.z += bv.z; v.w += bv.w;
        if (g.relu) { v.x = v.x > 0.f ? v.x : 0.f; v.y = v.y > 0.f ? v.y : 0.f; v.z = v.z > 0.f ? v.z : 0.f; v.w = v.w > 0.f ? v.w : 0.f; }
        *reinterpret_cast<float4*>(g.C + row * g.ldc + col) = v;
      }
    }
    asm volatile("s_waitcnt lgkmcnt(0)" ::: "memory");
  }
}

__global__ void __launch_bounds__(256)
k_gemm3_reduce(const float* __restrict__ partial, int splits, int64_t M, int64_t N, float* __restrict__ out, int64_t ldc) {
  const int64_t n4 = N >> 2;
  const int64_t total = M * n4;
  for (int64_t i = (int64_t)blockIdx.x * blockDim.x + threadIdx.x; i < total; i += (int64_t)gridDim.x * blockDim.x) {
    const int64_t row = i / n4, c4 = i - row * n4;
    float4 s = make_float4(0.f, 0.f, 0.f, 0.f);
    for (int k = 0; k < splits; ++k) {
      const float4 v = *reinterpret_cast<const float4*>(partial + ((int64_t)k * M + row) * N + c4 * 4);
      s.x += v.x; s.y += v.y; s.z += v.z; s.w += v.w;
    }
    *reinterpret_cast<float4*>(out + row * ldc + c4 * 4) = s;
  }
}

__global__ void __launch_bounds__(256)
k_g3_head_reduce(const float* __restrict__ part, int ncb, int64_t M, int O, const float* __restrict__ bias2,
                 float* __restrict__ out, int64_t ldo) {
  for (int64_t i = (int64_t)blockIdx.x * 256 + threadIdx.x; i < M * 2; i += (int64_t)gridDim.x * 256) {
    const int64_t row = i >> 1;
    const int half = (int)(i & 1);
    float4 sum = make_float4(0.f, 0.f, 0.f, 0.f);
    for (int cb = 0; cb < ncb; ++cb) {
      const float4 v = *reinterpret_cast<const float4*>(part + ((int64_t)cb * M + row) * 8 + half * 4);
      sum.x += v.x; sum.y += v.y; sum.z += v.z; sum.w += v.w;
    }
    const float r[4] = {sum.x, sum.y, sum.z, sum.w};
#pragma unroll
    for (int e = 0; e < 4; ++e) {
      const int o = half * 4 + e;
      if (o < O) out[row * ldo + o] = r[e] + (bias2 ? bias2[o] : 0.f);
    }
  }
}

static int g_g3_mid_mode = -1;

static int g3_splits(int64_t M, int64_t N, int64_t K) {
  const int64_t tiles = ((M + 255) / 256) * ((N + 255) / 256);
  int64_t s = 8 * ((256 + 8 * tiles - 1) / (8 * tiles));
  const int64_t nk = K / 16;
  while (s > 8 && nk / s < 64) s -= 8;
  return (int)s;
}

}

extern "C" int mirl_gemm3_supported(int32_t layout, int64_t M, int64_t N, int64_t K) {
  if (layout < 0 || layout > 2) return 0;
  if (M < 1 || N < 1 || K < 16 || (K % 16)) return 0;
  if (M >= (1LL << 31) || N >= (1LL << 31)) return 0;
  if (layout == 2) {
    if (N % 4) return 0;
    if (K / 16 < 8) return 0;
  }
  return 1;
}

extern "C" int mirl_gemm3_workspace_bytes(int32_t layout, int64_t M, int64_t N, int64_t K, int64_t* bytes) {
  using namespace mirl;
  if (!bytes) return fail(MIRL_ERR_ARG, "gemm3_workspace_bytes: null out");
  if (!mirl_gemm3_supported(layout, M, N, K)) return fail(MIRL_ERR_ARG, "gemm3: unsupported layout / shape");
  *bytes = layout == 2 ? (int64_t)g3_splits(M, N, K) * M * N * (int64_t)sizeof(float) : 0;
  return MIRL_OK;
}

namespace mirl {
struct G3Opt {
  const float* mul = nullptr; int64_t ldmul = 0; int32_t mul_shift = 0;
  float* pre = nullptr; int64_t ldpre = 0;
  const float* w2 = nullptr; float* part = nullptr;
  float* gsum = nullptr; int64_t ldgsum = 0;
};

struct G3Kernel { const void* fn; const char* name; };
static G3Kernel g3_kernel(int layout, int vec, bool mul, bool w2, bool gsum, bool narrow) {
  static const void* const plain[4][2] = {{(const void*)k_gemm3<true, true, 0, false>, (const void*)k_gemm3<true, true, 0, true>},
                                          {(const void*)k_gemm3<true, false, 0, false>, (const void*)k_gemm3<true, false, 0, true>},
                                          {nullptr , (const void*)k_gemm3<false, false, 0, true>},
                                          {(const void*)k_gemm3<true, true, 1, false>, (const void*)k_gemm3<true, true, 1, true>}};
  static const char* const names[4] = {"k_gemm3_nt", "k_gemm3_nn", "k_gemm3_tn", "k_gemm3_nt_mul"};
  if (gsum) return {(const void*)k_gemm3<true, false, 3, true>, "k_gemm3_nn_qp"};
  if (w2) return {(const void*)k_gemm3<true, true, 2, true>, "k_gemm3_nt_head"};
  if (narrow) return {(const void*)k_gemm3<false, false, 0, true, true>, "k_gemm3_tn"};
  const int which = mul ? 3 : layout;
  return {plain[which][vec], names[which]};
}
}

static int g3_launch(int32_t layout, int64_t M, int64_t N, int64_t K, const float* A, int64_t lda, const float* B,
                     int64_t ldb, float* C, int64_t ldc, const float* bias, int32_t relu, void* workspace,
                     int64_t workspace_bytes, void* stream, const mirl::G3Opt& o = mirl::G3Opt()) {
  using namespace mirl;
  if (!mirl_gemm3_supported(layout, M, N, K)) return fail(MIRL_ERR_ARG, "gemm3: unsupported layout / shape");
  if (!A || !B || (!C && !o.w2)) return fail(MIRL_ERR_ARG, "gemm3: null operand");
  const bool akc = layout != 2, bkc = layout == 0;
  if (akc && ((lda % 4) || !aligned16(A) || lda < K)) return fail(MIRL_ERR_ARG, "gemm3: A must be 16-byte aligned with lda % 4 == 0");
  if (bkc && ((ldb % 4) || !aligned16(B) || ldb < K)) return fail(MIRL_ERR_ARG, "gemm3: B must be 16-byte aligned with ldb % 4 == 0");
  if (!akc && lda < M) return fail(MIRL_ERR_ARG, "gemm3: lda < M");
  if (!bkc && ldb < N) return fail(MIRL_ERR_ARG, "gemm3: ldb < N");
  if (ldc < N) return fail(MIRL_ERR_ARG, "gemm3: ldc < N");
  if (layout == 2 && (bias || relu)) return fail(MIRL_ERR_ARG, "gemm3: no epilogue with split K");
  hipStream_t st = (hipStream_t)stream;
  G3Args g;
  g.A = A; g.B = B; g.C = C; g.bias = bias; g.M = M; g.N = N; g.K = K; g.lda = lda; g.ldb = ldb; g.ldc = ldc;
  g.relu = relu ? 1 : 0;
  g.mul = o.mul; g.ldmul = o.ldmul; g.mul_shift = o.mul_shift; g.pre = o.pre; g.ldpre = o.ldpre;
  g.w2 = o.w2; g.part = o.part; g.gsum = o.gsum; g.ldgsum = o.ldgsum;
  g.vec_ok = (N % 4 == 0) && (ldc % 4 == 0) && aligned16(C, o.w2, bias, o.mul, o.pre) && (!o.mul || o.ldmul % 4 == 0) && (!o.pre || o.ldpre % 4 == 0);
  g.mt = (int)((M + 255) / 256); g.nt = (int)((N + 255) / 256);
  g.splits = 1; g.steps_per_split = (int)(K / 16);
  unsigned grid = (unsigned)(8 * ((g.mt + 7) / 8) * g.nt);
  if (K <= 128) {
    const unsigned resident = (unsigned)(cu_count() / 8 * 8);
    if (resident && grid > resident) grid = resident;
  }
  if (layout == 2) {
    g.splits = g3_splits(M, N, K);
    const int64_t need = (int64_t)g.splits * M * N * (int64_t)sizeof(float);
    if (!workspace || workspace_bytes < need || (ldc % 4) || !aligned16(workspace, C))
      return fail(MIRL_ERR_ARG, "gemm3: split-K workspace too small / misaligned");
    g.steps_per_split = (int)((K / 16 + g.splits - 1) / g.splits);
    g.C = (float*)workspace; g.ldc = N;
    grid = (unsigned)(g.mt * g.nt * g.splits);
  }
  const int vec = g.vec_ok ? 1 : 0;
  const double flop = 2.0 * (double)M * (double)N * (double)K;
  if (g_g3_mid_mode != 0 && layout == 0 && !o.mul && !o.w2 && !o.gsum && vec && (N % 4) == 0 && (int64_t)g.mt * g.nt < 192 && N > 128 &&
      ((int64_t)g.mt * ((N + G3M_BROWS - 1) / G3M_BROWS) >= 192 || (int64_t)g.mt * g.nt < 24)) {
    if (int rc = raise_lds_limit(k_gemm3_mid, G3M_LDS)) return rc;
    g.nt = (int)((N + G3M_BROWS - 1) / G3M_BROWS);
    const unsigned mgrid = (unsigned)(8 * ((g.mt + 7) / 8) * g.nt);
    ProfScope ps("k_gemm3_nt_mid", 4.0 * ((double)M * K + (double)N * K + (double)M * N), st, flop);
    void* kargs[] = {(void*)&g};
    MIRL_HIP(hipLaunchKernel((const void*)k_gemm3_mid, dim3(mgrid), dim3(512), kargs, G3M_LDS, st));
    return MIRL_OK;
  }
  if (o.gsum) {
    if (!vec || layout != 1 || !o.mul || o.mul_shift != 5 || !o.pre || !o.part || (o.ldgsum % 4) || !aligned16(o.gsum, o.part) || (M % 32))
      return fail(MIRL_ERR_ARG, "gemm3: the fused feature-product backward needs the NN form, groups of 32 rows and 16-byte aligned rows");
  } else if (o.w2) {
    if (!vec || layout != 0 || o.mul || !o.part) return fail(MIRL_ERR_ARG, "gemm3: the fused following layer needs the NT form with 16-byte aligned rows");
  }
  const G3Kernel k = g3_kernel(layout, vec, o.mul, o.w2, o.gsum, layout == 2 && N <= 64);
  if (int rc = raise_lds_limit(k.fn, G3_LDS)) return rc;
  {
    double bytes = 4.0 * ((double)M * K + (double)N * K + (double)M * N * (layout == 2 ? (double)g.splits : 1.0));
    if (o.mul) bytes += 4.0 * ((o.pre ? (double)M * N : 0.0) + (double)(M >> o.mul_shift) * N * (o.gsum ? 2.0 : 1.0));
    if (o.w2) bytes += 4.0 * (8.0 * (double)N + 8.0 * (double)M * (double)((N + 63) / 64)) - (C ? 0.0 : 4.0 * (double)M * N);
    ProfScope ps(k.name, bytes, st, flop);
    void* kargs[] = {(void*)&g};
    MIRL_HIP(hipLaunchKernel(k.fn, dim3(grid), dim3(512), kargs, G3_LDS, st));
  }
  if (layout == 2) {
    ProfScope ps("k_gemm3_reduce", (double)(g.splits + 1) * (double)M * (double)N * 4.0, st);
    hipLaunchKernelGGL(k_gemm3_reduce, dim3(capped_grid((M * (N / 4) + 255) / 256, 4096)), dim3(256), 0, st, (const float*)workspace, g.splits, M, N, C, ldc);
    MIRL_LAUNCH_CHECK();
  }
  return MIRL_OK;
}

extern "C" int mirl_gemm3(int32_t layout, int64_t M, int64_t N, int64_t K, const float* A, int64_t lda, const float* B,
                          int64_t ldb, float* C, int64_t ldc, const float* bias, int32_t relu, void* workspace,
                          int64_t workspace_bytes, void* stream) {
  return g3_launch(layout, M, N, K, A, lda, B, ldb, C, ldc, bias, relu, workspace, workspace_bytes, stream);
}

extern "C" int mirl_gemm3_mid_set(int32_t mode) {
  if (mode < -1 || mode > 1) return mirl::fail(MIRL_ERR_ARG, "gemm3_mid_set: mode is -1 (default), 0 or 1");
  mirl::g_g3_mid_mode = mode;
  return MIRL_OK;
}

extern "C" int mirl_gemm3_nt_mul(int64_t M, int64_t N, int64_t K, const float* A, int64_t lda, const float* B, int64_t ldb,
                                 float* C, int64_t ldc, const float* bias, int32_t relu, const float* mul, int64_t ldmul,
                                 int32_t group_shift, float* pre, int64_t ldpre, void* stream) {
  using namespace mirl;
  if (!mul || group_shift < 0 || group_shift > 30 || ldmul < N || (pre && ldpre < N))
    return fail(MIRL_ERR_ARG, "gemm3_nt_mul: bad multiplier / pre-activation arguments");
  G3Opt o;
  o.mul = mul; o.ldmul = ldmul; o.mul_shift = group_shift; o.pre = pre; o.ldpre = ldpre;
  return g3_launch(0, M, N, K, A, lda, B, ldb, C, ldc, bias, relu, nullptr, 0, stream, o);
}

extern "C" int mirl_gemm3_nn_qp_partial_rows(int64_t M, int64_t* rows) {
  if (!rows || M < 1) return mirl::fail(MIRL_ERR_ARG, "gemm3_nn_qp_partial_rows: M >= 1");
  *rows = 2 * ((M + 255) / 256);
  return MIRL_OK;
}

extern "C" int mirl_gemm3_nn_qp(int64_t M, int64_t N, int64_t K, const float* A, int64_t lda, const float* B, int64_t ldb,
                                const float* emb, int64_t ldemb, const float* x, int64_t ldx, float* d_pre, int64_t ldd,
                                float* dx, int64_t lddx, float* db_partial, void* stream) {
  using namespace mirl;
  if (!emb || !x || !d_pre || !dx || !db_partial || ldemb < N || ldx < N || lddx < N || (ldemb % 4) || !aligned16(emb))
    return fail(MIRL_ERR_ARG, "gemm3_nn_qp: bad embedding / feature / output arguments");
  G3Opt o;
  o.mul = x; o.ldmul = ldx; o.mul_shift = 5; o.pre = const_cast<float*>(emb); o.ldpre = ldemb;
  o.part = db_partial; o.gsum = dx; o.ldgsum = lddx;
  return g3_launch(1, M, N, K, A, lda, B, ldb, d_pre, ldd, nullptr, 0, nullptr, 0, stream, o);
}

extern "C" int mirl_gemm3_head_workspace_bytes(int64_t M, int64_t N, int64_t* bytes) {
  if (!bytes || M < 1 || N < 1) return mirl::fail(MIRL_ERR_ARG, "bad gemm3_head_workspace_bytes arguments");
  *bytes = 8 * (int64_t)sizeof(float) * M * ((N + 255) / 256 * 4);
  return MIRL_OK;
}

extern "C" int mirl_gemm3_nt_head(int64_t M, int64_t N, int64_t K, const float* A, int64_t lda, const float* B, int64_t ldb,
                                  float* C, int64_t ldc, const float* bias, int32_t relu, const float* w2, int32_t O,
                                  const float* bias2, float* out2, int64_t ldo, void* workspace, int64_t workspace_bytes,
                                  void* stream) {
  using namespace mirl;
  int64_t need = 0;
  if (O < 1 || O > 8 || !w2 || !out2 || ldo < O || !workspace || mirl_gemm3_head_workspace_bytes(M, N, &need) || workspace_bytes < need ||
      !aligned16(workspace) || (N % 4))
    return fail(MIRL_ERR_ARG, "bad gemm3_nt_head arguments (1 <= O <= 8, N % 4 == 0, 16-byte aligned workspace of head_workspace_bytes)");
  if (!C) ldc = N;
  G3Opt o;
  o.w2 = w2; o.part = (float*)workspace;
  if (int rc = g3_launch(0, M, N, K, A, lda, B, ldb, C, ldc, bias, relu, nullptr, 0, stream, o)) return rc;
  const int ncb = (int)((N + 255) / 256 * 4);
  hipStream_t st = (hipStream_t)stream;
  ProfScope ps("k_g3_head_reduce", 4.0 * (8.0 * ncb + O) * (double)M, st);
  hipLaunchKernelGGL(k_g3_head_reduce, dim3(capped_grid((2 * M + 255) / 256, 16384)), dim3(256), 0, st, (const float*)workspace, ncb, M, (int)O, bias2, out2, ldo);
  MIRL_LAUNCH_CHECK();
  return MIRL_OK;
}
```

rltime_amd/models/torch/fused.py:

```python
import ctypes as C
import importlib
import os

import torch
import torch.nn.functional as F


from . import gemm3

_QP_EPILOGUE = True
_CONV3 = os.environ.get("MIRL_CONV3", "1") != "0"
_CONV3_MIN_WORK = 400000000


def _lib():
    return importlib.import_module("rltime_amd._lib")


_floats = {}


def _scratch_floats(query):
    if query not in _floats:
        L = _lib()
        n = C.c_int64()
        L.check(getattr(L.lib, query)(C.byref(n)), query)
        _floats[query] = n.value
    return _floats[query]


def _pow2_quads(c):
    q = c // 4
    return c % 4 == 0 and 1 <= q <= 256 and 256 % q == 0


def _fusable(*tensors):
    return all(t.is_cuda and t.dtype == torch.float32 for t in tensors) and not torch.is_autocast_enabled()


def bias_relu_rows_(y, bias, channels):
    L = _lib()
    L.check(L.lib.mirl_bias_relu_rows(y.numel() // channels, channels, L.ptr(y), L.ptr(bias), L.stream()), "mirl_bias_relu_rows")
    return y


def relu_bwd_bias_rows(dy, y, channels):
    L = _lib()
    if dy.data_ptr() % 16:
        dy = dy.clone()
    rows = y.numel() // channels
    blocks = C.c_int32()
    L.check(L.lib.mirl_colsum_blocks(rows, channels, C.byref(blocks)))
    g = torch.empty_like(y)
    db = torch.empty(channels, dtype=torch.float32, device=y.device)
    partial = torch.empty((blocks.value, channels), dtype=torch.float32, device=y.device)
    L.check(L.lib.mirl_relu_bwd_bias_rows(rows, channels, L.ptr(dy), L.ptr(y), L.ptr(g), L.ptr(db), L.ptr(partial), blocks.value,
                                          L.stream()), "mirl_relu_bwd_bias_rows")
    return g, db


class _LinearReLU(torch.autograd.Function):
    @staticmethod
    def forward(ctx, x, weight, bias):
        out = gemm3.linear_fwd(x, weight, bias, relu=True)
        ctx.save_for_backward(x, weight, out)
        return out

    @staticmethod
    def backward(ctx, grad):
        x, weight, out = ctx.saved_tensors
        n = out.shape[1]
        if _pow2_quads(n) and out.is_contiguous():
            g, db = relu_bwd_bias_rows(grad.contiguous(), out, n)
        else:
            g = torch.ops.aten.threshold_backward(grad.contiguous(), out, 0.0)
            db = g.sum(0) if ctx.needs_input_grad[2] else None
        dx = gemm3.grad_input(g, weight) if ctx.needs_input_grad[0] else None
        dw = gemm3.grad_weight(g, x) if ctx.needs_input_grad[1] else None
        return dx, dw, (db if ctx.needs_input_grad[2] else None)


def linear_relu(x, weight, bias):
    if x.dim() == 2 and x.dtype == weight.dtype and _fusable(x, weight):
        return _LinearReLU.apply(x, weight, bias)
    return F.relu(F.linear(x, weight, bias))


def conv3_supported(x, weight, stride, min_work=None):
    if not (_CONV3 and x.is_cuda and x.dtype == torch.float32 and weight.dtype == torch.float32 and x.dim() == 4
            and x.is_contiguous(memory_format=torch.channels_last) and x.data_ptr() % 16 == 0
            and stride[0] == stride[1]):
        return False
    n, c, h, w = x.shape
    f, _, kh, kw = weight.shape
    s = int(stride[0])
    if h < kh or w < kw:
        return False
    work = n * ((h - kh) // s + 1) * ((w - kw) // s + 1) * f * c * kh * kw
    return work >= (_CONV3_MIN_WORK if min_work is None else min_work) and bool(_lib().lib.mirl_conv3_fwd_supported(c, f, kh, kw, s, h, w))


def conv3_bias_relu(x, weight, bias, stride, relu=True):
    L = _lib()
    n, c, h, w = x.shape
    f, _, kh, kw = weight.shape
    s = int(stride[0])
    wk = weight.permute(0, 2, 3, 1)
    if not wk.is_contiguous():
        wk = wk.contiguous()
    y = torch.empty((n, f, (h - kh) // s + 1, (w - kw) // s + 1), dtype=torch.float32, device=x.device,
                    memory_format=torch.channels_last)
    b = bias.contiguous() if bias is not None else None
    L.check(L.lib.mirl_conv3_fwd(n, h, w, c, f, kh, kw, s, L.ptr(x), L.ptr(wk), L.ptr(b),
                                 1 if relu else 0, L.ptr(y), L.stream()), "mirl_conv3_fwd")
    return y


def act_conv_layer(x, weight, bias, stride):
    if not (x.is_cuda and x.dim() == 4 and x.dtype == torch.float32 and weight.dtype == torch.float32 and bias is not None
            and x.is_contiguous(memory_format=torch.channels_last) and weight.is_contiguous(memory_format=torch.channels_last)
            and stride[0] == stride[1] and weight.shape[2] == weight.shape[3] and bias.is_contiguous()
            and x.data_ptr() % 16 == 0 and weight.data_ptr() % 16 == 0 and x.shape[0] > 0):
        return 0
    f, c, k, _ = weight.shape
    layer = 2 if (c, k, int(stride[0])) == (32, 4, 2) else 3 if (c, k, int(stride[0])) == (64, 3, 1) else 0
    if layer and _lib().lib.mirl_act_conv_supported(layer, c, f, k, int(stride[0]), x.shape[2], x.shape[3]):
        return layer
    return 0


def act_conv_bias_relu(layer, x, weight, bias, stride):
    L = _lib()
    n, c, h, w = x.shape
    f, _, k, _ = weight.shape
    s = int(stride[0])
    ho, wo = (h - k) // s + 1, (w - k) // s + 1
    y = torch.empty((n, f, ho, wo), dtype=torch.float32, device=x.device, memory_format=torch.channels_last)
    L.check(L.lib.mirl_act_conv_fwd(layer, n, h, w, L.ptr(x), L.ptr(weight), L.ptr(bias), L.ptr(y), ho * wo * f, L.stream()), "mirl_act_conv_fwd")
    return y


class _ConvBiasReLU(torch.autograd.Function):
    @staticmethod
    def forward(ctx, x, weight, bias, stride, track=True):
        layer = 0
        if conv3_supported(x, weight, stride):
            y = conv3_bias_relu(x, weight, bias, stride)
        elif not (track and any(ctx.needs_input_grad)) and (layer := act_conv_layer(x, weight, bias, stride)):
            y = act_conv_bias_relu(layer, x, weight, bias, stride)
        else:
            y = F.conv2d(x, weight, None, stride)
            if not y.is_contiguous(memory_format=torch.channels_last):
                y = y.contiguous(memory_format=torch.channels_last)
            bias_relu_rows_(y, bias, y.shape[1])
        ctx.stride = stride
        ctx.save_for_backward(x, weight, y)
        return y

    @staticmethod
    def backward(ctx, grad):
        x, weight, y = ctx.saved_tensors
        c = y.shape[1]
        grad = grad.contiguous(memory_format=torch.channels_last)
        if _pow2_quads(c):
            g, db = relu_bwd_bias_rows(grad, y, c)
        else:
            g = torch.ops.aten.threshold_backward(grad, y, 0.0)
            db = g.sum((0, 2, 3))
        need_x, need_w = ctx.needs_input_grad[0], ctx.needs_input_grad[1]
        dx = dw = None
        if need_w and conv_wrw_supported(x, weight, ctx.stride, g):
            dw = conv_wgrad_b3(g, x, weight, ctx.stride)
            need_w = False
        if need_x and _CONV2_BWD and g.shape[0] and conv2_bwd_data_supported(x, weight, ctx.stride, g):
            dx = conv2_bwd_data(g, weight, x)
            need_x = False
        if need_x and _CONV3_BWD and g.shape[0] and conv3_bwd_data_supported(x, weight, ctx.stride, g):
            dx = conv3_bwd_data(g, weight, x)
            need_x = False
        lib_dx, lib_dw, _ = torch.ops.aten.convolution_backward(
            g, x, weight, None, list(ctx.stride), [0, 0], [1, 1], False, [0, 0], 1, [need_x, need_w, False]) \
            if (need_x or need_w) else (None, None, None)
        return (dx if dx is not None else lib_dx), (dw if dw is not None else lib_dw), \
            (db if ctx.needs_input_grad[2] else None), None, None


_CONV2_BWD = True
_CONV_WRW = True
_CONV_WRW_MIN_WORK = 1 << 31
_wrw_scratch = {}


def conv_wrw_supported(x, weight, stride, g, min_work=None):
    if not (_CONV_WRW and x.is_cuda and x.dtype == torch.float32 and g.dtype == torch.float32 and weight.dtype == torch.float32
            and x.dim() == 4 and stride[0] == stride[1] and g.shape[0] > 0
            and x.is_contiguous(memory_format=torch.channels_last) and g.is_contiguous(memory_format=torch.channels_last)
            and x.data_ptr() % 16 == 0 and g.data_ptr() % 16 == 0 and not torch.is_autocast_enabled()):
        return False
    n, c, h, w = x.shape
    f, _, kh, kw = weight.shape
    work = g.shape[0] * g.shape[2] * g.shape[3] * f * c * kh * kw
    if work < (_CONV_WRW_MIN_WORK if min_work is None else min_work):
        return False
    return bool(_lib().lib.mirl_conv_wrw_b3_supported(c, f, kh, kw, int(stride[0]), h, w))


def conv_wgrad_b3(g, x, weight, stride):
    L = _lib()
    n, c, h, w = x.shape
    f, _, kh, kw = weight.shape
    key = (x.device.index, torch.cuda.current_stream().cuda_stream, c, f, kh, kw)
    scratch = _wrw_scratch.get(key)
    if scratch is None:
        nbytes = C.c_int64()
        L.check(L.lib.mirl_conv_wrw_b3_scratch_bytes(c, f, kh, kw, C.byref(nbytes)), "mirl_conv_wrw_b3_scratch_bytes")
        scratch = _wrw_scratch[key] = torch.empty(nbytes.value, dtype=torch.uint8, device=x.device)
    dw = torch.empty((f, kh, kw, c), dtype=torch.float32, device=x.device)
    L.check(L.lib.mirl_conv_wrw_b3(n, h, w, c, f, kh, kw, int(stride[0]), L.ptr(x), L.ptr(g), L.ptr(scratch), scratch.numel(), L.ptr(dw),
                                   L.stream()), "mirl_conv_wrw_b3")
    return dw.permute(0, 3, 1, 2)


def conv2_bwd_data_supported(x, weight, stride, g):
    if not (g.is_contiguous(memory_format=torch.channels_last) and g.data_ptr() % 16 == 0
            and tuple(stride) == (2, 2) and weight.shape[2] == weight.shape[3]):
        return False
    return bool(_lib().lib.mirl_conv2_bwd_data_supported(weight.shape[1], weight.shape[0], weight.shape[2], 2, x.shape[2],
                                                         x.shape[3], g.shape[2], g.shape[3]))


_CONV3_BWD = True


def conv3_bwd_data_supported(x, weight, stride, g):
    if not (g.is_contiguous(memory_format=torch.channels_last) and g.data_ptr() % 16 == 0 and g.dtype == torch.float32
            and tuple(stride) == (1, 1) and weight.shape[2] == weight.shape[3] and not torch.is_autocast_enabled()):
        return False
    return bool(_lib().lib.mirl_conv3_bwd_data_supported(weight.shape[1], weight.shape[0], weight.shape[2], 1, x.shape[2],
                                                         x.shape[3], g.shape[2], g.shape[3]))


def conv3_bwd_data(g, weight, x_like):
    L = _lib()
    dx = torch.empty_like(x_like, memory_format=torch.channels_last)
    wpk = torch.empty(_scratch_floats("mirl_conv3_bwd_data_wpk_floats"), dtype=torch.float32, device=g.device)
    so, sc, sh, sw = weight.stride()
    L.check(L.lib.mirl_conv3_bwd_data(g.shape[0], g.shape[2], g.shape[3], L.ptr(g), L.ptr(weight), so, sc, sh, sw, L.ptr(wpk), wpk.numel(),
                                      L.ptr(dx), L.stream()), "mirl_conv3_bwd_data")
    return dx


_CONV2_BWD_PIPE = 1


def conv2_bwd_data(g, weight, x_like):
    L = _lib()
    dx = torch.empty_like(x_like, memory_format=torch.channels_last)
    wpk = torch.empty(_scratch_floats("mirl_conv2_bwd_data_wpk_floats"), dtype=torch.float32, device=g.device)
    so, sc, sh, sw = weight.stride()
    L.check(L.lib.mirl_conv2_bwd_data_ex(g.shape[0], g.shape[2], g.shape[3], L.ptr(g), L.ptr(weight), so, sc, sh, sw, L.ptr(wpk), wpk.numel(),
                                         L.ptr(dx), _CONV2_BWD_PIPE, L.stream()), "mirl_conv2_bwd_data_ex")
    return dx


def conv_bias_relu(x, conv):
    if (_fusable(x, conv.weight) and conv.bias is not None and conv.padding == (0, 0) and conv.dilation == (1, 1)
            and conv.groups == 1 and x.dim() == 4 and x.is_contiguous(memory_format=torch.channels_last)
            and conv.weight.is_contiguous(memory_format=torch.channels_last)):
        return _ConvBiasReLU.apply(x, conv.weight, conv.bias, tuple(conv.stride), torch.is_grad_enabled())
    return F.relu(conv(x))


def frames_to_f32_nhwc(x, scale):
    L = _lib()
    n, c, h, w = x.shape
    out = torch.empty((n, c, h, w), dtype=torch.float32, device=x.device, memory_format=torch.channels_last)
    L.check(L.lib.mirl_frames_to_f32_nhwc(n, c, h * w, L.ptr(x), float(scale), L.ptr(out), L.stream()), "mirl_frames_to_f32_nhwc")
    return out


def conv_u8_supported(x, conv):
    if not (isinstance(x, torch.Tensor) and x.is_cuda and x.dtype == torch.uint8 and x.dim() == 4 and x.is_contiguous()
            and x.data_ptr() % 16 == 0 and conv.bias is not None and conv.weight.dtype == torch.float32
            and conv.padding == (0, 0) and conv.dilation == (1, 1) and conv.groups == 1
            and conv.kernel_size[0] == conv.kernel_size[1] and conv.stride[0] == conv.stride[1]
            and conv.in_channels == x.shape[1] and not torch.is_autocast_enabled()):
        return False
    return bool(_lib().lib.mirl_conv1_u8_supported(x.shape[1], x.shape[2], x.shape[3], conv.out_channels,
                                                   conv.kernel_size[0], conv.stride[0]))


class _ConvU8BiasReLU(torch.autograd.Function):
    @staticmethod
    def forward(ctx, x, weight, bias, scale, stride):
        L = _lib()
        n, _, h, w = x.shape
        f, k = weight.shape[0], weight.shape[2]
        oh, ow = (h - k) // stride + 1, (w - k) // stride + 1
        y = torch.empty((n, f, oh, ow), dtype=torch.float32, device=x.device, memory_format=torch.channels_last)
        if n:
            wpk = torch.empty(_scratch_floats("mirl_conv1_u8_wpk_floats"), dtype=torch.float32, device=x.device)
            so, sc, sh, sw = weight.stride()
            b = bias if bias.data_ptr() % 16 == 0 else bias.clone()
            L.check(L.lib.mirl_conv1_u8_fwd(n, h, w, L.ptr(x), L.ptr(weight), so, sc, sh, sw, L.ptr(b), float(scale), L.ptr(wpk), L.ptr(y),
                                            L.stream()), "mirl_conv1_u8_fwd")
        ctx.scale = scale
        ctx.save_for_backward(x, weight, y)
        return y

    @staticmethod
    def backward(ctx, grad):
        x, weight, y = ctx.saved_tensors
        grad = grad.contiguous(memory_format=torch.channels_last)
        if not (ctx.needs_input_grad[1] and x.shape[0]):
            _, db = relu_bwd_bias_rows(grad, y, y.shape[1])
            dw = torch.zeros_like(weight) if ctx.needs_input_grad[1] else None
            return None, dw, (db if ctx.needs_input_grad[2] else None), None, None
        L = _lib()
        n, _, h, w = x.shape
        scratch = torch.empty(_scratch_floats("mirl_conv1_u8_wrw_scratch_floats"), dtype=torch.float32, device=x.device)
        dw = torch.empty_like(weight)
        so, sc, sh, sw = dw.stride()
        if grad.data_ptr() % 16 == 0:
            db = torch.empty(weight.shape[0], dtype=torch.float32, device=x.device)
            L.check(L.lib.mirl_conv1_u8_wrw_masked(n, h, w, L.ptr(x), L.ptr(grad), L.ptr(y), float(ctx.scale), L.ptr(scratch), L.ptr(dw), so, sc, sh, sw,
                                                   L.ptr(db), L.stream()), "mirl_conv1_u8_wrw_masked")
        else:
            g, db = relu_bwd_bias_rows(grad, y, y.shape[1])
            L.check(L.lib.mirl_conv1_u8_wrw(n, h, w, L.ptr(x), L.ptr(g), float(ctx.scale), L.ptr(scratch), L.ptr(dw), so, sc, sh, sw,
                                            L.stream()), "mirl_conv1_u8_wrw")
        return None, dw, (db if ctx.needs_input_grad[2] else None), None, None


def conv_u8_bias_relu(x, conv, scale):
    return _ConvU8BiasReLU.apply(x, conv.weight, conv.bias, float(scale), int(conv.stride[0]))


def cos_embed(taus, freq):
    D = freq.shape[0]
    if D % 4 == 0 and _fusable(taus, freq) and taus.is_contiguous():
        L = _lib()
        out = torch.empty((taus.shape[0], D), dtype=torch.float32, device=taus.device)
        L.check(L.lib.mirl_cos_embed(taus.shape[0], D, L.ptr(taus), L.ptr(freq), L.ptr(out), L.stream()), "mirl_cos_embed")
        return out
    return torch.cos(freq * taus.unsqueeze(1))


class _QPLink:
    __slots__ = ("out", "x", "emb", "n", "done", "placeholder", "__weakref__")


_qp_links = {}


def _qp_announce(out, x, emb, n):
    import weakref
    link = _QPLink()
    link.out, link.x, link.emb, link.n, link.done, link.placeholder = weakref.ref(out), x, emb, n, None, None
    if len(_qp_links) > 16:
        for k in [k for k, v in _qp_links.items() if v() is None or v().out() is None]:
            del _qp_links[k]
    _qp_links[out.data_ptr()] = weakref.ref(link)
    return link


def _qp_find(x):
    ref = _qp_links.get(x.data_ptr())
    link = ref() if ref is not None else None
    out = link.out() if link is not None else None
    if out is None or not (x is out or x._base is out) or x.shape != out.shape or not x.is_contiguous() or x._version != out._version:
        return None
    return link


class _QuantileProduct(torch.autograd.Function):

    @staticmethod
    def forward(ctx, x, phi, weight, bias, n, track=True):
        L = _lib()
        M, Cf = x.shape
        need = track and any(ctx.needs_input_grad)
        if _QP_EPILOGUE and gemm3.quantile_product_supported(x, phi, weight, bias, n):
            out, emb = gemm3.quantile_product(x, phi, weight, bias, n, need)
        else:
            emb = torch._addmm_activation(bias, phi, weight.t(), use_gelu=False)
            out = torch.empty_like(emb) if need else emb
            L.check(L.lib.mirl_iqn_mul_fwd(M, n, Cf, L.ptr(x), L.ptr(emb), L.ptr(out), L.stream()), "mirl_iqn_mul_fwd")
        ctx.n = n
        ctx.save_for_backward(x, phi, weight, emb)
        ctx.link = _qp_announce(out, x, emb, n) if need else None
        return out

    @staticmethod
    def backward(ctx, grad):
        L = _lib()
        x, phi, weight, emb = ctx.saved_tensors
        M, Cf = x.shape
        link = getattr(ctx, "link", None)
        done, fused = (link.done, link.placeholder) if link is not None else (None, None)
        if link is not None:
            link.done = link.placeholder = None
        only_placeholder = done is not None and grad.data_ptr() == fused.data_ptr() and all(s == 0 for s in grad.stride())
        if done is None or not only_placeholder:
            grad = grad.contiguous()
            if _pow2_quads(Cf):
                blocks = min(M, 2048)
                d_pre = torch.empty_like(emb)
                dx = torch.empty_like(x)
                db = torch.empty(Cf, dtype=torch.float32, device=x.device)
                partial = torch.empty((blocks, Cf), dtype=torch.float32, device=x.device)
                L.check(L.lib.mirl_iqn_mul_bwd(M, ctx.n, Cf, L.ptr(grad), L.ptr(emb), L.ptr(x), L.ptr(d_pre), L.ptr(dx), L.ptr(db), L.ptr(partial),
                                               blocks, L.stream()), "mirl_iqn_mul_bwd")
            else:
                g3, e3 = grad.view(M, ctx.n, Cf), emb.view(M, ctx.n, Cf)
                dx = (g3 * e3).sum(1)
                d_pre = (g3 * x.unsqueeze(1)).masked_fill_(e3 <= 0, 0.0).view(M * ctx.n, Cf)
                db = d_pre.sum(0)
            if done is not None:
                d_pre += done[0]
                dx += done[1]
                db += done[2]
        else:
            d_pre, dx, db = done
        dw = gemm3.grad_weight(d_pre, phi) if ctx.needs_input_grad[2] else None
        return (dx if ctx.needs_input_grad[0] else None), None, dw, (db if ctx.needs_input_grad[3] else None), None, None


def quantile_product(x, phi, weight, bias, n):
    if x.dim() == 2 and _fusable(x, phi, weight) and x.is_contiguous() and phi.is_contiguous() and not phi.requires_grad:
        if _pow2_quads(x.shape[1]) or (_QP_EPILOGUE and gemm3.quantile_product_supported(x, phi, weight, bias, n)):
            return _QuantileProduct.apply(x, phi, weight, bias, n, torch.is_grad_enabled())
    emb = linear_relu(phi, weight, bias)
    return (x.unsqueeze(1) * emb.reshape(x.shape[0], n, -1)).reshape(x.shape[0] * n, -1)


class _DuelingTail(torch.autograd.Function):

    @staticmethod
    def forward(ctx, x, w1, b1, wo, bo, wv, bv, wq, bq, track=True):
        h1 = w1.shape[0]
        wj, bj = gemm3.joint_rows((w1, wv)), gemm3.joint_rows((b1, bv))
        na, nv = wo.shape[0], wq.shape[0]
        w2 = gemm3.joint_blockdiag((wo, wq)) if (na + nv <= 8 and wo.shape[1] == h1) else None
        if w2 is not None and gemm3.head_supported(x, wj, bj, w2):
            keep = bool(track) and any(ctx.needs_input_grad)
            both, out = gemm3.linear_relu_head(x, wj, bj, w2, gemm3.joint_rows((bo, bq)), keep)
            a, v = out[:, :na], out[:, na:]
        else:
            both = gemm3.linear_fwd(x, wj, bj, relu=True)
            a = torch.addmm(bo, both[:, :h1], wo.t())
            v = torch.addmm(bq, both[:, h1:], wq.t())
        ctx.h1 = h1
        ctx.link = _qp_find(x) if (track and ctx.needs_input_grad[0]) else None
        ctx.save_for_backward(x, w1, wo, wv, wq, both)
        return a, v

    @staticmethod
    def backward(ctx, ga, gv):
        x, w1, wo, wv, wq, both = ctx.saved_tensors
        h1 = ctx.h1
        ga, gv = ga.contiguous(), gv.contiguous()
        width = both.shape[1]
        dwo_dwq = None
        if (_pow2_quads(width) and h1 % 4 == 0 and ga.shape[1] <= 16 and gv.shape[1] <= 16
                and wo.is_contiguous() and wq.is_contiguous()):
            L = _lib()
            M = both.shape[0]
            blocks = C.c_int32()
            L.check(L.lib.mirl_colsum_blocks(M, width, C.byref(blocks)))
            g = torch.empty_like(both)
            db = torch.empty(width, dtype=torch.float32, device=both.device)
            partial = torch.empty((blocks.value, width), dtype=torch.float32, device=both.device)
            kw = max(ga.shape[1], gv.shape[1])
            if kw <= 8:
                dwj = torch.empty((kw, width), dtype=torch.float32, device=both.device)
                partial_w = torch.empty((blocks.value, kw, width), dtype=torch.float32, device=both.device)
                L.check(L.lib.mirl_dueling_tail_bwd_w(M, h1, width - h1, ga.shape[1], gv.shape[1], L.ptr(ga), L.ptr(gv), L.ptr(wo), L.ptr(wq),
                                                      L.ptr(both), L.ptr(g), L.ptr(db), L.ptr(partial), blocks.value, L.ptr(dwj), L.ptr(partial_w),
                                                      L.stream()), "mirl_dueling_tail_bwd_w")
                dwo_dwq = (dwj[:ga.shape[1], :h1], dwj[:gv.shape[1], h1:])
            else:
                L.check(L.lib.mirl_dueling_tail_bwd(M, h1, width - h1, ga.shape[1], gv.shape[1], L.ptr(ga), L.ptr(gv), L.ptr(wo), L.ptr(wq),
                                                    L.ptr(both), L.ptr(g), L.ptr(db), L.ptr(partial), blocks.value, L.stream()),
                        "mirl_dueling_tail_bwd")
        else:
            d_both = torch.empty_like(both)
            torch.mm(ga, wo, out=d_both[:, :h1])
            torch.mm(gv, wq, out=d_both[:, h1:])
            if _pow2_quads(width):
                g, db = relu_bwd_bias_rows(d_both, both, width)
            else:
                g = torch.ops.aten.threshold_backward(d_both, both, 0.0)
                db = g.sum(0)
        g1, g2 = g[:, :h1], g[:, h1:]
        dx = None
        wj = gemm3.joint_rows((w1, wv)) if gemm3.enabled() else None
        if wj is not None and gemm3.supported(gemm3.NN, g, wj) and gemm3.supported(gemm3.TN, g, x):
            link = getattr(ctx, "link", None)
            if ctx.needs_input_grad[0] and link is not None and gemm3.grad_input_qp_supported(g, wj, link.emb, link.x, link.n):
                link.done = gemm3.grad_input_qp(g, wj, link.emb, link.x)
                link.placeholder = dx = torch.zeros(1, dtype=x.dtype, device=x.device).expand(x.shape)
            elif ctx.needs_input_grad[0]:
                dx = gemm3.gemm(gemm3.NN, g, wj)
            dwj = gemm3.gemm(gemm3.TN, g, x)
            dw1, dwv = dwj[:h1], dwj[h1:]
        else:
            if ctx.needs_input_grad[0]:
                dx = g1.mm(w1)
                dx.addmm_(g2, wv)
            dw1, dwv = g1.t().mm(x), g2.t().mm(x)
        if dwo_dwq is not None:
            dwo, dwq = dwo_dwq
        else:
            dwo = ga.t().mm(both[:, :h1])
            dwq = gv.t().mm(both[:, h1:])
        return dx, dw1, db[:h1], dwo, ga.sum(0), dwv, db[h1:], dwq, gv.sum(0), None


def dueling_tail(x, fc, out_layer, value_hidden, value_layer):
    if x.dim() == 2 and _fusable(x, fc.weight) and x.is_contiguous():
        return _DuelingTail.apply(x, fc.weight, fc.bias, out_layer.weight, out_layer.bias,
                                  value_hidden.weight, value_hidden.bias, value_layer.weight, value_layer.bias,
                                  torch.is_grad_enabled())
    h = F.relu(fc(x))
    return out_layer(h), value_layer(F.relu(value_hidden(x)))
```

rltime_amd/models/torch/gemm3.py:

```python
import ctypes as C
import importlib
import os

import torch

NT, NN, TN = 0, 1, 2
_MIN_WORK = 1 << 31
_MIN_AREA = 6000000
_ws = {}


def _lib():
    return importlib.import_module("rltime_amd._lib")


def enabled():
    return os.environ.get("MIRL_GEMM3", "1") != "0"


def _rowmajor(t):
    return t.dim() == 2 and t.stride(1) == 1 and t.stride(0) >= t.shape[1] and t.dtype == torch.float32 and t.is_cuda


def supported(layout, a, b, min_work=None):
    if not (_rowmajor(a) and _rowmajor(b)):
        return False
    if layout == NT:
        M, K, N = a.shape[0], a.shape[1], b.shape[0]
        ok = b.shape[1] == K and a.stride(0) % 4 == 0 and b.stride(0) % 4 == 0 and a.data_ptr() % 16 == 0 and b.data_ptr() % 16 == 0
    elif layout == NN:
        M, K, N = a.shape[0], a.shape[1], b.shape[1]
        ok = b.shape[0] == K and a.stride(0) % 4 == 0 and a.data_ptr() % 16 == 0
    else:
        K, M, N = a.shape[0], a.shape[1], b.shape[1]
        ok = b.shape[0] == K
    floor = _MIN_WORK if min_work is None else min_work
    if not ok or M * N * K < floor or (floor > 0 and layout != TN and M * N < _MIN_AREA):
        return False
    return bool(_lib().lib.mirl_gemm3_supported(layout, M, N, K))


def _workspace(device, nbytes):
    key = (device.index, torch.cuda.current_stream().cuda_stream)
    buf = _ws.get(key)
    if buf is None or buf.numel() < nbytes:
        buf = torch.empty(max(nbytes, 1), dtype=torch.uint8, device=device)
        _ws[key] = buf
    return buf


REFRESH_ALWAYS = False
_joint = {}


def joint_rows(tensors):
    key = tuple(t.data_ptr() for t in tensors)
    vers = tuple(t._version for t in tensors)
    hit = _joint.get(key)
    if hit is not None and hit[0] == vers and not REFRESH_ALWAYS:
        return hit[1]
    with torch.no_grad():
        if hit is not None and hit[1].shape[0] == sum(t.shape[0] for t in tensors):
            out = hit[1]
            torch.cat([t.detach() for t in tensors], 0, out=out)
        else:
            out = torch.cat([t.detach() for t in tensors], 0)
    if len(_joint) > 32:
        _joint.clear()
    _joint[key] = (vers, out, tensors)
    return out


def gemm(layout, a, b, bias=None, relu=False, out=None):
    L = _lib()
    if layout == NT:
        M, K, N = a.shape[0], a.shape[1], b.shape[0]
    elif layout == NN:
        M, K, N = a.shape[0], a.shape[1], b.shape[1]
    else:
        K, M, N = a.shape[0], a.shape[1], b.shape[1]
    if out is None:
        out = torch.empty((M, N), dtype=torch.float32, device=a.device)
    ws, wsb = None, 0
    if layout == TN:
        need = C.c_int64()
        L.check(L.lib.mirl_gemm3_workspace_bytes(layout, M, N, K, C.byref(need)), "mirl_gemm3_workspace_bytes")
        wsb = need.value
        ws = _workspace(a.device, wsb)
    L.check(L.lib.mirl_gemm3(layout, M, N, K, L.ptr(a), a.stride(0), L.ptr(b), b.stride(0), L.ptr(out), out.stride(0),
                             L.ptr(bias), 1 if relu else 0, L.ptr(ws), wsb, L.stream()), "mirl_gemm3")
    return out



def linear_fwd(x, w, bias=None, relu=False):
    if enabled() and supported(NT, x, w) and (bias is None or (bias.is_contiguous() and bias.dtype == torch.float32)):
        return gemm(NT, x, w, bias, relu)
    if relu:
        return torch._addmm_activation(bias, x, w.t(), use_gelu=False) if bias is not None else torch.relu(x.mm(w.t()))
    return torch.addmm(bias, x, w.t()) if bias is not None else x.mm(w.t())


def grad_input(g, w):
    if enabled() and supported(NN, g, w):
        return gemm(NN, g, w)
    return g.mm(w)


def grad_weight(g, x):
    if enabled() and supported(TN, g, x):
        return gemm(TN, g, x)
    return g.t().mm(x)


_QP_BWD = True


def grad_input_qp_supported(g, w, emb, x, n):
    return (_QP_BWD and enabled() and n == 32 and supported(NN, g, w) and _rowmajor(emb) and _rowmajor(x)
            and emb.shape == (g.shape[0], w.shape[1]) and x.shape == (g.shape[0] // 32, w.shape[1]) and g.shape[0] % 32 == 0
            and w.shape[1] % 4 == 0 and emb.stride(0) % 4 == 0 and x.stride(0) % 4 == 0
            and emb.data_ptr() % 16 == 0 and x.data_ptr() % 16 == 0)


def grad_input_qp(g, w, emb, x):
    L = _lib()
    M, N = g.shape
    K = w.shape[1]
    rows = C.c_int64()
    L.check(L.lib.mirl_gemm3_nn_qp_partial_rows(M, C.byref(rows)), "mirl_gemm3_nn_qp_partial_rows")
    d_pre = torch.empty((M, K), dtype=torch.float32, device=g.device)
    dx = torch.empty((M // 32, K), dtype=torch.float32, device=g.device)
    part = torch.empty((rows.value, K), dtype=torch.float32, device=g.device)
    L.check(L.lib.mirl_gemm3_nn_qp(M, K, N, L.ptr(g), g.stride(0), L.ptr(w), w.stride(0), L.ptr(emb), emb.stride(0), L.ptr(x), x.stride(0),
                                   L.ptr(d_pre), d_pre.stride(0), L.ptr(dx), dx.stride(0), L.ptr(part), L.stream()), "mirl_gemm3_nn_qp")
    return d_pre, dx, part.sum(0)


class _Linear(torch.autograd.Function):
    @staticmethod
    def forward(ctx, x, w, bias):
        ctx.save_for_backward(x, w)
        return linear_fwd(x, w, bias)

    @staticmethod
    def backward(ctx, g):
        x, w = ctx.saved_tensors
        g = g.contiguous()
        dx = grad_input(g, w) if ctx.needs_input_grad[0] else None
        dw = grad_weight(g, x) if ctx.needs_input_grad[1] else None
        db = g.sum(0) if ctx.needs_input_grad[2] else None
        return dx, dw, db


def linear(x, w, bias):
    if enabled() and x.dim() == 2 and supported(NT, x, w) and bias is not None:
        return _Linear.apply(x, w, bias.contiguous())
    return torch.nn.functional.linear(x, w, bias)


def quantile_product_supported(x, phi, weight, bias, n):
    return (enabled() and n > 0 and (n & (n - 1)) == 0 and supported(NT, phi, weight) and _rowmajor(x)
            and x.shape[1] == weight.shape[0] and x.shape[0] * n == phi.shape[0]
            and bias is not None and bias.is_contiguous() and bias.dtype == torch.float32)


def quantile_product(x, phi, weight, bias, n, keep_embedding):
    L = _lib()
    R, K, N = phi.shape[0], phi.shape[1], weight.shape[0]
    out = torch.empty((R, N), dtype=torch.float32, device=phi.device)
    emb = torch.empty((R, N), dtype=torch.float32, device=phi.device) if keep_embedding else None
    L.check(L.lib.mirl_gemm3_nt_mul(R, N, K, L.ptr(phi), phi.stride(0), L.ptr(weight), weight.stride(0), L.ptr(out), out.stride(0),
                                    L.ptr(bias), 1, L.ptr(x), x.stride(0), n.bit_length() - 1,
                                    L.ptr(emb), N, L.stream()), "mirl_gemm3_nt_mul")
    return out, emb


_HEAD = True


def head_supported(x, w, bias, w2):
    return (_HEAD and enabled() and supported(NT, x, w) and bias is not None and bias.is_contiguous() and bias.dtype == torch.float32
            and w.shape[0] % 4 == 0 and _rowmajor(w2) and w2.is_contiguous() and w2.shape[1] == w.shape[0] and 1 <= w2.shape[0] <= 8)


def linear_relu_head(x, w, bias, w2, bias2, keep_hidden):
    L = _lib()
    M, K, N, O = x.shape[0], x.shape[1], w.shape[0], w2.shape[0]
    pad = joint_pad8(w2)
    hidden = torch.empty((M, N), dtype=torch.float32, device=x.device) if keep_hidden else None
    out = torch.empty((M, O), dtype=torch.float32, device=x.device)
    need = C.c_int64()
    L.check(L.lib.mirl_gemm3_head_workspace_bytes(M, N, C.byref(need)), "mirl_gemm3_head_workspace_bytes")
    ws = _workspace(x.device, need.value)
    L.check(L.lib.mirl_gemm3_nt_head(M, N, K, L.ptr(x), x.stride(0), L.ptr(w), w.stride(0), L.ptr(hidden), N,
                                     L.ptr(bias), 1, L.ptr(pad), O, L.ptr(bias2), L.ptr(out), O,
                                     L.ptr(ws), need.value, L.stream()), "mirl_gemm3_nt_head")
    return hidden, out


_pad8 = {}


def joint_pad8(w2):
    key = (w2.data_ptr(), tuple(w2.shape))
    hit = _pad8.get(key)
    if hit is not None and hit[0] == w2._version and hit[2].untyped_storage().data_ptr() == w2.untyped_storage().data_ptr() \
            and not REFRESH_ALWAYS:
        return hit[1]
    with torch.no_grad():
        pad = hit[1] if hit is not None else torch.zeros((8, w2.shape[1]), dtype=torch.float32, device=w2.device)
        pad[:w2.shape[0]].copy_(w2.detach())
    if len(_pad8) > 32:
        _pad8.clear()
    _pad8[key] = (w2._version, pad, w2.detach())
    return pad


def joint_blockdiag(blocks):
    key = tuple(t.data_ptr() for t in blocks)
    vers = tuple(t._version for t in blocks)
    hit = _joint.get(("bd",) + key)
    if hit is not None and hit[0] == vers and not REFRESH_ALWAYS:
        return hit[1]
    with torch.no_grad():
        out = hit[1] if hit is not None else torch.zeros((sum(t.shape[0] for t in blocks), sum(t.shape[1] for t in blocks)),
                                                          dtype=torch.float32, device=blocks[0].device)
        r = c = 0
        for t in blocks:
            out[r:r + t.shape[0], c:c + t.shape[1]].copy_(t.detach())
            r, c = r + t.shape[0], c + t.shape[1]
    _joint[("bd",) + key] = (vers, out, blocks)
    return out
```

Before: 485,000.

## Fuse ReLU-backward mask and bias-grad reduction into consumer data-grad kernels

Adds masked variants of the conv3 backward-data kernel and the NN GEMM backward that apply the ReLU mask of the producing layer and accumulate its bias-gradient column sums in the epilogue. A Python link mechanism lets the producing conv layer find and reuse the already-masked gradient, skipping its separate relu_bwd_bias pass. This removes a full read/write pass over the gradient activations. In exchange it adds bookkeeping through weakref links and version checks, plus an extra small reduction kernel.

```diff
diff --git a/include/mirl.h b/include/mirl.h
--- a/include/mirl.h
+++ b/include/mirl.h
@@ -223,6 +223,10 @@
 int mirl_conv3_bwd_data_wpk_floats(int64_t* floats);
 int mirl_conv3_bwd_data(int64_t N, int32_t OH, int32_t OW, const float* g, const float* weight, int64_t ws_o,
                         int64_t ws_c, int64_t ws_h, int64_t ws_w, float* wpk, int64_t wpk_floats, float* dx, void* stream);
+int mirl_conv3_bwd_data_masked_parts(int64_t N, int32_t* parts);
+int mirl_conv3_bwd_data_masked(int64_t N, int32_t OH, int32_t OW, const float* g, const float* weight, int64_t ws_o,
+                               int64_t ws_c, int64_t ws_h, int64_t ws_w, float* wpk, int64_t wpk_floats, const float* x,
+                               float* dx, float* part, int32_t parts, float* db, void* stream);
 
 int mirl_gemm3_supported(int32_t layout, int64_t M, int64_t N, int64_t K);
 int mirl_gemm3_workspace_bytes(int32_t layout, int64_t M, int64_t N, int64_t K, int64_t* bytes);
@@ -242,6 +246,10 @@
 int mirl_gemm3_nn_qp(int64_t M, int64_t N, int64_t K, const float* A, int64_t lda, const float* B, int64_t ldb,
                      const float* emb, int64_t ldemb, const float* x, int64_t ldx, float* d_pre, int64_t ldd,
                      float* dx, int64_t lddx, float* db_partial, void* stream);
+int mirl_gemm3_nn_relu_supported(int64_t M, int64_t N, int64_t K, int64_t ldy, int64_t ldc);
+int mirl_gemm3_nn_relu_partial_rows(int64_t M, int64_t* rows);
+int mirl_gemm3_nn_relu(int64_t M, int64_t N, int64_t K, const float* A, int64_t lda, const float* B, int64_t ldb,
+                       const float* y, int64_t ldy, float* C, int64_t ldc, float* part, float* db, void* stream);
 
 int mirl_conv3_fwd_supported(int32_t C, int32_t F, int32_t KH, int32_t KW, int32_t S, int32_t H, int32_t W);
 int mirl_conv3_fwd(int64_t N, int32_t H, int32_t W, int32_t C, int32_t F, int32_t KH, int32_t KW, int32_t S,
diff --git a/rltime_amd/_lib.py b/rltime_amd/_lib.py
--- a/rltime_amd/_lib.py
+++ b/rltime_amd/_lib.py
@@ -174,6 +174,8 @@
     "mirl_conv3_bwd_data_supported": [_i32, _i32, _i32, _i32, _i32, _i32, _i32, _i32],
     "mirl_conv3_bwd_data_wpk_floats": [_P(_i64)],
     "mirl_conv3_bwd_data": [_i64, _i32, _i32, _vp, _vp, _i64, _i64, _i64, _i64, _vp, _i64, _vp, _vp],
+    "mirl_conv3_bwd_data_masked_parts": [_i64, _P(_i32)],
+    "mirl_conv3_bwd_data_masked": [_i64, _i32, _i32, _vp, _vp, _i64, _i64, _i64, _i64, _vp, _i64, _vp, _vp, _vp, _i32, _vp, _vp],
     "mirl_conv2_bwd_data_ex": [_i64, _i32, _i32, _vp, _vp, _i64, _i64, _i64, _i64, _vp, _i64, _vp, _i32, _vp],
     "mirl_conv3_fwd_supported": [_i32, _i32, _i32, _i32, _i32, _i32, _i32],
     "mirl_conv3_fwd": [_i64, _i32, _i32, _i32, _i32, _i32, _i32, _i32, _vp, _vp, _vp, _i32, _vp, _vp],
@@ -186,6 +188,9 @@
     "mirl_gemm3_nt_mul": [_i64, _i64, _i64, _vp, _i64, _vp, _i64, _vp, _i64, _vp, _i32, _vp, _i64, _i32, _vp, _i64, _vp],
     "mirl_gemm3_nn_qp_partial_rows": [_i64, _P(_i64)],
     "mirl_gemm3_nn_qp": [_i64, _i64, _i64, _vp, _i64, _vp, _i64, _vp, _i64, _vp, _i64, _vp, _i64, _vp, _i64, _vp, _vp],
+    "mirl_gemm3_nn_relu_supported": [_i64, _i64, _i64, _i64, _i64],
+    "mirl_gemm3_nn_relu_partial_rows": [_i64, _P(_i64)],
+    "mirl_gemm3_nn_relu": [_i64, _i64, _i64, _vp, _i64, _vp, _i64, _vp, _i64, _vp, _i64, _vp, _vp, _vp],
     "mirl_gemm3_head_workspace_bytes": [_i64, _i64, _P(_i64)],
     "mirl_gemm3_nt_head": [_i64, _i64, _i64, _vp, _i64, _vp, _i64, _vp, _i64, _vp, _i32, _vp, _i32, _vp, _vp, _i64, _vp, _i64, _vp],
     "mirl_act_conv_supported": [_i32, _i32, _i32, _i32, _i32, _i32, _i32],
diff --git a/rltime_amd/csrc/conv_mid.hip b/rltime_amd/csrc/conv_mid.hip
--- a/rltime_amd/csrc/conv_mid.hip
+++ b/rltime_amd/csrc/conv_mid.hip
@@ -270,10 +270,10 @@
   wpk3[(slot * 3 + 2) * 64 + lane] = make_uint4(l0.x, l0.y, l1.x, l1.y);
 }
 
-template <int FPI>
-__global__ void __launch_bounds__(512) __attribute__((amdgpu_waves_per_eu(2, 2)))
-k_conv3_bwd_data_b3(int N, int OH, int OW, unsigned iw_magic, const float* __restrict__ g, const uint4* __restrict__ wpk3,
-                    float* __restrict__ dx) {
+template <int FPI, bool MASK>
+__device__ __forceinline__ void c3b_bwd_data(int N, int OH, int OW, unsigned iw_magic, const float* __restrict__ g,
+                                             const uint4* __restrict__ wpk3, float* __restrict__ dx, const float* __restrict__ xin,
+                                             float* __restrict__ part) {
   extern __shared__ __align__(16) char c3b_lds[];
   const int tid = threadIdx.x, lane = tid & 63, wave = __builtin_amdgcn_readfirstlane(tid >> 6);
   const int ct = wave >> 1, kh2 = wave & 1;
@@ -297,6 +297,7 @@
   for (int o = tid; o < 3 * plane / 16; o += 512) reinterpret_cast<uint4*>(c3b_lds)[o] = make_uint4(0u, 0u, 0u, 0u);
   const int units = (N + FPI - 1) / FPI;
   bool first = true;
+  g3_f32x4 colsum = {0.f, 0.f, 0.f, 0.f};
   for (int u0 = blockIdx.x; u0 < units; u0 += gridDim.x) {
     const int n0 = u0 * FPI;
     const int frames = N - n0 < FPI ? N - n0 : FPI;
@@ -334,6 +335,17 @@
     }
     __syncthreads();
     const int pend = frames * IHW;
+    [[maybe_unused]] const int64_t e0 = (int64_t)n0 * IHW * C3B_C + 16 * ct + 4 * kq;
+    [[maybe_unused]] g3_f32x4 xv[(C3B_MAXT + 1) / 2];
+    if constexpr (MASK) {
+#pragma unroll
+      for (int t = 0; t < C3B_MAXT; ++t) {
+        if ((t & 1) == kh2 && t * 16 < pend) {
+          const int p = t * 16 + j, pc = p < pend ? p : pend - 1;
+          xv[t >> 1] = *reinterpret_cast<const g3_f32x4*>(xin + e0 + (int64_t)pc * C3B_C);
+        }
+      }
+    }
     g3_f32x4 acc[C3B_MAXT];
 #pragma unroll
     for (int t = 0; t < C3B_MAXT; ++t) {
@@ -366,21 +378,90 @@
     }
     __syncthreads();
     g3_f32x4* xb = reinterpret_cast<g3_f32x4*>(c3b_lds) + (ct * C3B_MAXT) * 64 + lane;
-    if (kh2 == 1) {
-#pragma unroll
-      for (int t = 0; t < C3B_MAXT; ++t) if (t * 16 < pend) xb[t * 64] = acc[t];
-    }
-    __syncthreads();
-    if (kh2 == 0) {
+    if constexpr (!MASK) {
+      if (kh2 == 1) {
+#pragma unroll
+        for (int t = 0; t < C3B_MAXT; ++t) if (t * 16 < pend) xb[t * 64] = acc[t];
+      }
+      __syncthreads();
+      if (kh2 == 0) {
+#pragma unroll
+        for (int t = 0; t < C3B_MAXT; ++t) {
+          const int p = t * 16 + j;
+          if (p < pend) {
+            const int f = p / IHW, r = p - f * IHW;
+            *reinterpret_cast<g3_f32x4*>(dx + ((int64_t)(n0 + f) * IHW + r) * C3B_C + 16 * ct + 4 * kq) = acc[t] + xb[t * 64];
+          }
+        }
+      }
+    } else {
+#pragma unroll
+      for (int t = 0; t < C3B_MAXT; ++t) if ((t & 1) != kh2 && t * 16 < pend) xb[t * 64] = acc[t];
+      __syncthreads();
 #pragma unroll
       for (int t = 0; t < C3B_MAXT; ++t) {
         const int p = t * 16 + j;
-        if (p < pend) {
-          const int f = p / IHW, r = p - f * IHW;
-          *reinterpret_cast<g3_f32x4*>(dx + ((int64_t)(n0 + f) * IHW + r) * C3B_C + 16 * ct + 4 * kq) = acc[t] + xb[t * 64];
-        }
-      }
-    }
+        if ((t & 1) == kh2 && p < pend) {
+          g3_f32x4 v = acc[t] + xb[t * 64];
+          const g3_f32x4 xx = xv[t >> 1];
+          v.x = xx.x > 0.f ? v.x : 0.f; v.y = xx.y > 0.f ? v.y : 0.f; v.z = xx.z > 0.f ? v.z : 0.f; v.w = xx.w > 0.f ? v.w : 0.f;
+          *reinterpret_cast<g3_f32x4*>(dx + e0 + (int64_t)p * C3B_C) = v;
+          colsum = colsum + v;
+        }
+      }
+    }
+  }
+  if constexpr (MASK) {
+    __syncthreads();
+    g3_f32x4* red = reinterpret_cast<g3_f32x4*>(c3b_lds);
+    red[wave * 64 + lane] = colsum;
+    __syncthreads();
+    if (tid < C3B_C) {
+      const int rct = tid >> 4, rkq = (tid >> 2) & 3, e = tid & 3;
+      const float* rf = reinterpret_cast<const float*>(c3b_lds);
+      float s = 0.f;
+      for (int h = 0; h < 2; ++h)
+        for (int l = 0; l < 16; ++l) s = s + rf[(((rct * 2 + h) * 64) + rkq * 16 + l) * 4 + e];
+      part[(int64_t)blockIdx.x * C3B_C + tid] = s;
+    }
+  }
+}
+
+template <int FPI>
+__global__ void __launch_bounds__(512) __attribute__((amdgpu_waves_per_eu(2, 2)))
+k_conv3_bwd_data_b3(int N, int OH, int OW, unsigned iw_magic, const float* __restrict__ g, const uint4* __restrict__ wpk3,
+                    float* __restrict__ dx) {
+  c3b_bwd_data<FPI, false>(N, OH, OW, iw_magic, g, wpk3, dx, nullptr, nullptr);
+}
+
+template <int FPI>
+__global__ void __launch_bounds__(512) __attribute__((amdgpu_waves_per_eu(2, 2)))
+k_conv3_bwd_data_b3_masked(int N, int OH, int OW, unsigned iw_magic, const float* __restrict__ g, const uint4* __restrict__ wpk3,
+                           float* __restrict__ dx, const float* __restrict__ xin, float* __restrict__ part) {
+  c3b_bwd_data<FPI, true>(N, OH, OW, iw_magic, g, wpk3, dx, xin, part);
+}
+
+__global__ void __launch_bounds__(1024)
+k_conv3_bwd_db_reduce(const float* __restrict__ part, int rows, float* __restrict__ db) {
+  __shared__ float s_part[16][64];
+  const int lane = threadIdx.x & 63, w = threadIdx.x >> 6;
+  float s = 0.f;
+  int b = w;
+  for (; b + 7 * 16 < rows; b += 8 * 16) {
+    float v[8];
+#pragma unroll
+    for (int k = 0; k < 8; ++k) v[k] = part[(int64_t)(b + 16 * k) * C3B_C + lane];
+#pragma unroll
+    for (int k = 0; k < 8; ++k) s = s + v[k];
+  }
+  for (; b < rows; b += 16) s = s + part[(int64_t)b * C3B_C + lane];
+  s_part[w][lane] = s;
+  __syncthreads();
+  if (w == 0) {
+    float t = s_part[0][lane];
+#pragma unroll
+    for (int k = 1; k < 16; ++k) t = t + s_part[k][lane];
+    db[lane] = t;
   }
 }
 
@@ -504,3 +585,46 @@
   return bwd_data_launch<uint4>(c, k_conv3_pack_w3b, k_conv3_bwd_data_b3<2>, k_conv3_bwd_data_b3<1>, N, OH, OW, g, weight, ws_o, ws_c, ws_h, ws_w,
                                 wpk, dx, (hipStream_t)stream);
 }
+
+extern "C" int mirl_conv3_bwd_data_masked_parts(int64_t N, int32_t* parts) {
+  using namespace mirl;
+  if (N <= 0 || N >= (1LL << 30) || !parts) return fail(MIRL_ERR_ARG, "bad conv3_bwd_data_masked_parts arguments");
+  *parts = (int32_t)capped_grid(N, 256);
+  return MIRL_OK;
+}
+
+extern "C" int mirl_conv3_bwd_data_masked(int64_t N, int32_t OH, int32_t OW, const float* g, const float* weight, int64_t ws_o,
+                                          int64_t ws_c, int64_t ws_h, int64_t ws_w, float* wpk, int64_t wpk_floats, const float* x,
+                                          float* dx, float* part, int32_t parts, float* db, void* stream) {
+  using namespace mirl;
+  if (N <= 0 || N >= (1LL << 30) || !g || !weight || !wpk || !dx || !x || !part || !db) return fail(MIRL_ERR_ARG, "bad conv3_bwd_data_masked arguments");
+  if (wpk_floats < C3B_WPK_BYTES / 4) return fail(MIRL_ERR_ARG, "conv3_bwd_data_masked: wpk smaller than mirl_conv3_bwd_data_wpk_floats()");
+  if (!mirl_conv3_bwd_data_supported(C3B_C, C3B_F, C3B_K, 1, OH + 2, OW + 2, OH, OW)) return fail(MIRL_ERR_ARG, "conv3_bwd_data_masked: unsupported shape");
+  if (!aligned16(g, dx, wpk) || !aligned16(x, part)) return fail(MIRL_ERR_ARG, "conv3_bwd_data_masked: pointers must be 16-byte aligned");
+  hipStream_t st = (hipStream_t)stream;
+  const int IHW = (OH + 2) * (OW + 2);
+  const int fpi = (N >= 512 && 2 * IHW <= 16 * C3B_MAXT && c3b_lds_bytes(2, OH, OW) <= 150 * 1024) ? 2 : 1;
+  const unsigned grid = capped_grid((N + fpi - 1) / fpi, 256);
+  if ((int64_t)grid > parts) return fail(MIRL_ERR_ARG, "conv3_bwd_data_masked: part has fewer rows than workgroups");
+  {
+    ProfScope ps("k_conv3_pack_w3b", 4.0 * C3B_F * C3B_C * 9 + C3B_WPK_BYTES, st);
+    hipLaunchKernelGGL(k_conv3_pack_w3b, dim3((C3B_SLOTS * 64 + 255) / 256), dim3(256), 0, st, weight, ws_o, ws_c, ws_h, ws_w,
+                       reinterpret_cast<uint4*>(wpk));
+    MIRL_LAUNCH_CHECK();
+  }
+  const auto k = fpi == 2 ? k_conv3_bwd_data_b3_masked<2> : k_conv3_bwd_data_b3_masked<1>;
+  if (int rc = raise_lds_limit(k, 150 * 1024)) return rc;
+  {
+    ProfScope ps("k_conv3_bwd_data_b3", (double)N * 4.0 * C3B_F * ((double)OH * OW + 2.0 * IHW), st,
+                 (double)N * OH * OW * 2.0 * C3B_K * C3B_K * C3B_C * C3B_F);
+    hipLaunchKernelGGL(k, dim3(grid), dim3(512), c3b_lds_bytes(fpi, OH, OW), st, (int)N, OH, OW, magic_u32(OW + 2), g,
+                       reinterpret_cast<const uint4*>(wpk), dx, x, part);
+    MIRL_LAUNCH_CHECK();
+  }
+  {
+    ProfScope ps("k_conv3_bwd_db_reduce", (double)(grid + 1) * C3B_C * 4.0, st);
+    hipLaunchKernelGGL(k_conv3_bwd_db_reduce, dim3(1), dim3(1024), 0, st, part, (int)grid, db);
+    MIRL_LAUNCH_CHECK();
+  }
+  return MIRL_OK;
+}
diff --git a/rltime_amd/csrc/gemm3.hip b/rltime_amd/csrc/gemm3.hip
--- a/rltime_amd/csrc/gemm3.hip
+++ b/rltime_amd/csrc/gemm3.hip
@@ -283,6 +283,33 @@
           mg0 = *reinterpret_cast<const float4*>(g.mul + (r0 >> g.mul_shift) * g.ldmul + cc);
           mg1 = *reinterpret_cast<const float4*>(g.mul + (r1 >> g.mul_shift) * g.ldmul + cc);
         }
+        if (EP == 4) {
+          const int64_t cc = col < g.N ? col : 0;
+#pragma unroll
+          for (int gq = 0; gq < 2; ++gq) {
+            asm volatile("" ::: "memory");
+            g3_f32x4 yv[8];
+#pragma unroll
+            for (int u = 0; u < 8; ++u) {
+              const int64_t row = m0 + row_w + h * 64 + (gq * 8 + u) * 4 + (lane >> 4);
+              const int64_t rr = row < g.M ? row : g.M - 1;
+              yv[u] = __builtin_nontemporal_load(reinterpret_cast<const g3_f32x4*>(g.pre + rr * g.ldpre + cc));
+            }
+#pragma unroll
+            for (int u = 0; u < 8; ++u) {
+              const int rl = (gq * 8 + u) * 4 + (lane >> 4);
+              const int64_t row = m0 + row_w + h * 64 + rl;
+              const float4 t4 = *reinterpret_cast<const float4*>(tl + rl * G3_EPITCH + c4 * 4);
+              if (row < g.M && col < g.N) {
+                g3_f32x4 d = {t4.x, t4.y, t4.z, t4.w};
+                d.x = yv[u].x > 0.f ? d.x : 0.f; d.y = yv[u].y > 0.f ? d.y : 0.f;
+                d.z = yv[u].z > 0.f ? d.z : 0.f; d.w = yv[u].w > 0.f ? d.w : 0.f;
+                __builtin_nontemporal_store(d, reinterpret_cast<g3_f32x4*>(C + row * g.ldc + col));
+                sb += d;
+              }
+            }
+          }
+        }
         if (EP == 3) {
           const float4 mgs[2] = {mg0, mg1};
 #pragma unroll
@@ -327,7 +354,7 @@
         for (int q = 0; q < QN; ++q) {
           const int rl = q * 4 + (lane >> 4);
           const int64_t row = m0 + row_w + h * 64 + rl;
-          if (EP == 3) break;
+          if (EP == 3 || EP == 4) break;
           if (EP == 2 && !g.C) break;
           float4 v = *reinterpret_cast<const float4*>(tl + rl * G3_EPITCH + c4 * 4);
           if (row < g.M && col < g.N) {
@@ -347,7 +374,7 @@
         }
         asm volatile("s_waitcnt lgkmcnt(0)" ::: "memory");
       }
-      if (EP == 3) {
+      if (EP == 3 || EP == 4) {
 #pragma unroll
         for (int e = 0; e < 4; ++e) {
           float v = sb[e];
@@ -570,16 +597,18 @@
   float* pre = nullptr; int64_t ldpre = 0;
   const float* w2 = nullptr; float* part = nullptr;
   float* gsum = nullptr; int64_t ldgsum = 0;
+  bool mask = false;
 };
 
 struct G3Kernel { const void* fn; const char* name; };
-static G3Kernel g3_kernel(int layout, int vec, bool mul, bool w2, bool gsum, bool narrow) {
+static G3Kernel g3_kernel(int layout, int vec, bool mul, bool w2, bool gsum, bool narrow, bool mask) {
   static const void* const plain[4][2] = {{(const void*)k_gemm3<true, true, 0, false>, (const void*)k_gemm3<true, true, 0, true>},
                                           {(const void*)k_gemm3<true, false, 0, false>, (const void*)k_gemm3<true, false, 0, true>},
                                           {nullptr , (const void*)k_gemm3<false, false, 0, true>},
                                           {(const void*)k_gemm3<true, true, 1, false>, (const void*)k_gemm3<true, true, 1, true>}};
   static const char* const names[4] = {"k_gemm3_nt", "k_gemm3_nn", "k_gemm3_tn", "k_gemm3_nt_mul"};
   if (gsum) return {(const void*)k_gemm3<true, false, 3, true>, "k_gemm3_nn_qp"};
+  if (mask) return {(const void*)k_gemm3<true, false, 4, true>, "k_gemm3_nn"};
   if (w2) return {(const void*)k_gemm3<true, true, 2, true>, "k_gemm3_nt_head"};
   if (narrow) return {(const void*)k_gemm3<false, false, 0, true, true>, "k_gemm3_tn"};
   const int which = mul ? 3 : layout;
@@ -638,14 +667,18 @@
   if (o.gsum) {
     if (!vec || layout != 1 || !o.mul || o.mul_shift != 5 || !o.pre || !o.part || (o.ldgsum % 4) || !aligned16(o.gsum, o.part) || (M % 32))
       return fail(MIRL_ERR_ARG, "gemm3: the fused feature-product backward needs the NN form, groups of 32 rows and 16-byte aligned rows");
+  } else if (o.mask) {
+    if (!vec || layout != 1 || o.mul || o.w2 || !o.pre || !o.part || !aligned16(o.part))
+      return fail(MIRL_ERR_ARG, "gemm3: the fused ReLU backward needs the NN form with 16-byte aligned rows");
   } else if (o.w2) {
     if (!vec || layout != 0 || o.mul || !o.part) return fail(MIRL_ERR_ARG, "gemm3: the fused following layer needs the NT form with 16-byte aligned rows");
   }
-  const G3Kernel k = g3_kernel(layout, vec, o.mul, o.w2, o.gsum, layout == 2 && N <= 64);
+  const G3Kernel k = g3_kernel(layout, vec, o.mul, o.w2, o.gsum, layout == 2 && N <= 64, o.mask);
   if (int rc = raise_lds_limit(k.fn, G3_LDS)) return rc;
   {
     double bytes = 4.0 * ((double)M * K + (double)N * K + (double)M * N * (layout == 2 ? (double)g.splits : 1.0));
     if (o.mul) bytes += 4.0 * ((o.pre ? (double)M * N : 0.0) + (double)(M >> o.mul_shift) * N * (o.gsum ? 2.0 : 1.0));
+    if (o.mask) bytes += 4.0 * (double)M * N;
     if (o.w2) bytes += 4.0 * (8.0 * (double)N + 8.0 * (double)M * (double)((N + 63) / 64)) - (C ? 0.0 : 4.0 * (double)M * N);
     ProfScope ps(k.name, bytes, st, flop);
     void* kargs[] = {(void*)&g};
@@ -698,6 +731,61 @@
   o.mul = x; o.ldmul = ldx; o.mul_shift = 5; o.pre = const_cast<float*>(emb); o.ldpre = ldemb;
   o.part = db_partial; o.gsum = dx; o.ldgsum = lddx;
   return g3_launch(1, M, N, K, A, lda, B, ldb, d_pre, ldd, nullptr, 0, nullptr, 0, stream, o);
+}
+
+namespace mirl {
+__global__ void __launch_bounds__(1024)
+k_gemm3_colsum(const float* __restrict__ part, float* __restrict__ out, int rows, int64_t N) {
+  __shared__ float s_part[16][64];
+  const int lane = threadIdx.x & 63, w = threadIdx.x >> 6;
+  const int64_t c = (int64_t)blockIdx.x * 64 + lane;
+  float s = 0.f;
+  if (c < N) {
+    int b = w;
+    for (; b + 7 * 16 < rows; b += 8 * 16) {
+      float v[8];
+#pragma unroll
+      for (int k = 0; k < 8; ++k) v[k] = part[(int64_t)(b + 16 * k) * N + c];
+#pragma unroll
+      for (int k = 0; k < 8; ++k) s = s + v[k];
+    }
+    for (; b < rows; b += 16) s = s + part[(int64_t)b * N + c];
+  }
+  s_part[w][lane] = s;
+  __syncthreads();
+  if (w == 0 && c < N) {
+    float t = s_part[0][lane];
+#pragma unroll
+    for (int k = 1; k < 16; ++k) t = t + s_part[k][lane];
+    out[c] = t;
+  }
+}
+}
+
+extern "C" int mirl_gemm3_nn_relu_supported(int64_t M, int64_t N, int64_t K, int64_t ldy, int64_t ldc) {
+  return mirl_gemm3_supported(1, M, N, K) && (N % 4) == 0 && (ldy % 4) == 0 && (ldc % 4) == 0 && ldy >= N && ldc >= N ? 1 : 0;
+}
+
+extern "C" int mirl_gemm3_nn_relu_partial_rows(int64_t M, int64_t* rows) {
+  if (!rows || M < 1) return mirl::fail(MIRL_ERR_ARG, "gemm3_nn_relu_partial_rows: M >= 1");
+  *rows = 2 * ((M + 255) / 256);
+  return MIRL_OK;
+}
+
+extern "C" int mirl_gemm3_nn_relu(int64_t M, int64_t N, int64_t K, const float* A, int64_t lda, const float* B, int64_t ldb,
+                                  const float* y, int64_t ldy, float* C, int64_t ldc, float* part, float* db, void* stream) {
+  using namespace mirl;
+  if (!y || !C || !part || !db || !mirl_gemm3_nn_relu_supported(M, N, K, ldy, ldc) || !aligned16(y, C, part))
+    return fail(MIRL_ERR_ARG, "gemm3_nn_relu: bad activation / output arguments (N, ldy, ldc multiples of 4, 16-byte aligned)");
+  G3Opt o;
+  o.pre = const_cast<float*>(y); o.ldpre = ldy; o.part = part; o.mask = true;
+  if (int rc = g3_launch(1, M, N, K, A, lda, B, ldb, C, ldc, nullptr, 0, nullptr, 0, stream, o)) return rc;
+  hipStream_t st = (hipStream_t)stream;
+  const int rows = (int)(2 * ((M + 255) / 256));
+  ProfScope ps("k_gemm3_colsum", (double)(rows + 1) * (double)N * 4.0, st);
+  hipLaunchKernelGGL(k_gemm3_colsum, dim3((unsigned)((N + 63) / 64)), dim3(1024), 0, st, (const float*)part, db, rows, N);
+  MIRL_LAUNCH_CHECK();
+  return MIRL_OK;
 }
 
 extern "C" int mirl_gemm3_head_workspace_bytes(int64_t M, int64_t N, int64_t* bytes) {
diff --git a/rltime_amd/models/torch/fused.py b/rltime_amd/models/torch/fused.py
--- a/rltime_amd/models/torch/fused.py
+++ b/rltime_amd/models/torch/fused.py
@@ -155,6 +155,9 @@
             bias_relu_rows_(y, bias, y.shape[1])
         ctx.stride = stride
         ctx.save_for_backward(x, weight, y)
+        need = track and any(ctx.needs_input_grad)
+        ctx.in_link = _relu_find(x) if need and ctx.needs_input_grad[0] and _CONV3_BWD_MASK else None
+        ctx.link = _relu_announce(y) if need and _pow2_quads(y.shape[1]) else None
         return y
 
     @staticmethod
@@ -162,7 +165,14 @@
         x, weight, y = ctx.saved_tensors
         c = y.shape[1]
         grad = grad.contiguous(memory_format=torch.channels_last)
-        if _pow2_quads(c):
+        link = getattr(ctx, "link", None)
+        masked = None
+        if link is not None:
+            masked, link.done = link.done, None
+        if masked is not None and grad.data_ptr() == masked[0].data_ptr() and grad.numel() == masked[0].numel() \
+                and grad._version == masked[2]:
+            g, db = grad, masked[1]
+        elif _pow2_quads(c):
             g, db = relu_bwd_bias_rows(grad, y, c)
         else:
             g = torch.ops.aten.threshold_backward(grad, y, 0.0)
@@ -176,7 +186,12 @@
             dx = conv2_bwd_data(g, weight, x)
             need_x = False
         if need_x and _CONV3_BWD and g.shape[0] and conv3_bwd_data_supported(x, weight, ctx.stride, g):
-            dx = conv3_bwd_data(g, weight, x)
+            below = getattr(ctx, "in_link", None)
+            if below is not None:
+                dx, db_below = conv3_bwd_data_masked(g, weight, x)
+                below.done = (dx, db_below, dx._version)
+            else:
+                dx = conv3_bwd_data(g, weight, x)
             need_x = False
         lib_dx, lib_dw, _ = torch.ops.aten.convolution_backward(
             g, x, weight, None, list(ctx.stride), [0, 0], [1, 1], False, [0, 0], 1, [need_x, need_w, False]) \
@@ -248,6 +263,58 @@
     L.check(L.lib.mirl_conv3_bwd_data(g.shape[0], g.shape[2], g.shape[3], L.ptr(g), L.ptr(weight), so, sc, sh, sw, L.ptr(wpk), wpk.numel(),
                                       L.ptr(dx), L.stream()), "mirl_conv3_bwd_data")
     return dx
+
+
+def conv3_bwd_data_masked(g, weight, x):
+    L = _lib()
+    dx = torch.empty_like(x, memory_format=torch.channels_last)
+    wpk = torch.empty(_scratch_floats("mirl_conv3_bwd_data_wpk_floats"), dtype=torch.float32, device=g.device)
+    parts = C.c_int32()
+    L.check(L.lib.mirl_conv3_bwd_data_masked_parts(g.shape[0], C.byref(parts)), "mirl_conv3_bwd_data_masked_parts")
+    part = torch.empty((parts.value, 64), dtype=torch.float32, device=g.device)
+    db = torch.empty(64, dtype=torch.float32, device=g.device)
+    so, sc, sh, sw = weight.stride()
+    L.check(L.lib.mirl_conv3_bwd_data_masked(g.shape[0], g.shape[2], g.shape[3], L.ptr(g), L.ptr(weight), so, sc, sh, sw, L.ptr(wpk),
+                                             wpk.numel(), L.ptr(x), L.ptr(dx), L.ptr(part), parts.value, L.ptr(db), L.stream()),
+            "mirl_conv3_bwd_data_masked")
+    return dx, db
+
+
+_CONV3_BWD_MASK = True
+
+
+class _ReLULink:
+    __slots__ = ("out", "channels", "done", "__weakref__")
+
+
+_relu_links = {}
+
+
+def _relu_announce(y):
+    import weakref
+    link = _ReLULink()
+    link.out, link.channels, link.done = weakref.ref(y), y.shape[1], None
+    if len(_relu_links) > 16:
+        for k in [k for k, v in _relu_links.items() if v() is None or v().out() is None]:
+            del _relu_links[k]
+    _relu_links[y.data_ptr()] = weakref.ref(link)
+    return link
+
+
+def _relu_find(x):
+    ref = _relu_links.get(x.data_ptr())
+    link = ref() if ref is not None else None
+    return link if link is not None and _relu_link_holds(link, x) else None
+
+
+def _relu_link_holds(link, x):
+    out = link.out()
+    if (out is None or x.data_ptr() != out.data_ptr() or x.numel() != out.numel() or x._version != out._version
+            or x.dtype != torch.float32 or x.data_ptr() % 16 or not out.is_contiguous(memory_format=torch.channels_last)):
+        return False
+    if x.dim() == 4:
+        return x.shape == out.shape and x.stride() == out.stride()
+    return x.dim() == 2 and x.is_contiguous() and x.shape[0] == out.shape[0]
 
 
 _CONV2_BWD_PIPE = 1
diff --git a/rltime_amd/models/torch/gemm3.py b/rltime_amd/models/torch/gemm3.py
--- a/rltime_amd/models/torch/gemm3.py
+++ b/rltime_amd/models/torch/gemm3.py
@@ -137,25 +137,57 @@
     return d_pre, dx, part.sum(0)
 
 
+_RELU_BWD = True
+
+
+def grad_input_relu_supported(g, w, y):
+    return (_RELU_BWD and enabled() and supported(NN, g, w) and _rowmajor(y) and y.shape == (g.shape[0], w.shape[1])
+            and y.data_ptr() % 16 == 0
+            and bool(_lib().lib.mirl_gemm3_nn_relu_supported(g.shape[0], w.shape[1], g.shape[1], y.stride(0), w.shape[1])))
+
+
+def grad_input_relu(g, w, y):
+    L = _lib()
+    M, N = g.shape
+    K = w.shape[1]
+    rows = C.c_int64()
+    L.check(L.lib.mirl_gemm3_nn_relu_partial_rows(M, C.byref(rows)), "mirl_gemm3_nn_relu_partial_rows")
+    dx = torch.empty((M, K), dtype=torch.float32, device=g.device)
+    part = torch.empty((rows.value, K), dtype=torch.float32, device=g.device)
+    db = torch.empty(K, dtype=torch.float32, device=g.device)
+    L.check(L.lib.mirl_gemm3_nn_relu(M, K, N, L.ptr(g), g.stride(0), L.ptr(w), w.stride(0), L.ptr(y), y.stride(0), L.ptr(dx), dx.stride(0),
+                                     L.ptr(part), L.ptr(db), L.stream()), "mirl_gemm3_nn_relu")
+    return dx, db
+
+
 class _Linear(torch.autograd.Function):
     @staticmethod
-    def forward(ctx, x, w, bias):
+    def forward(ctx, x, w, bias, track=True):
         ctx.save_for_backward(x, w)
+        ctx.in_link = None
+        if _RELU_BWD and track and ctx.needs_input_grad[0]:
+            from . import fused
+            ctx.in_link = fused._relu_find(x)
         return linear_fwd(x, w, bias)
 
     @staticmethod
     def backward(ctx, g):
         x, w = ctx.saved_tensors
         g = g.contiguous()
-        dx = grad_input(g, w) if ctx.needs_input_grad[0] else None
+        below = getattr(ctx, "in_link", None)
+        if ctx.needs_input_grad[0] and below is not None and grad_input_relu_supported(g, w, x):
+            dx, db_cols = grad_input_relu(g, w, x)
+            below.done = (dx, db_cols.view(-1, below.channels).sum(0), dx._version)
+        else:
+            dx = grad_input(g, w) if ctx.needs_input_grad[0] else None
         dw = grad_weight(g, x) if ctx.needs_input_grad[1] else None
         db = g.sum(0) if ctx.needs_input_grad[2] else None
-        return dx, dw, db
+        return dx, dw, db, None
 
 
 def linear(x, w, bias):
     if enabled() and x.dim() == 2 and supported(NT, x, w) and bias is not None:
-        return _Linear.apply(x, w, bias.contiguous())
+        return _Linear.apply(x, w, bias.contiguous(), torch.is_grad_enabled())
     return torch.nn.functional.linear(x, w, bias)
 
 
```

New measurement: 488,100, median of 6. Within noise of the previous version (+0.6%).
